# ZJU-FAST-Lab/uneven_planner

Measured on AMD Instinct MI355X. Metric: MINCO traj-opts/sec (batch), higher is better.
Workload: dtype f64

## Files before the change

### include/uneven_hip.h

```cpp
#ifndef UNEVEN_HIP_H
#define UNEVEN_HIP_H

#include <stdint.h>

#ifdef __cplusplus
extern "C" {
#endif

typedef struct uph_map uph_map;
typedef struct uph_ctx uph_ctx;
typedef struct uph_kino uph_kino;
typedef struct uph_body_layer uph_body_layer;

#define UPH_OK 0
#define UPH_ERR_INVALID (-1)
#define UPH_ERR_HIP (-2)
#define UPH_ERR_NO_DEVICE (-3)
#define UPH_ERR_LIMIT (-4)
#define UPH_ERR_NO_CACHE (-5)

#define UPH_RET_STOPPED 3
#define UPH_RET_UNSUPPORTED 4

#define UPH_RET_LEFT_TILE 5
// ... 115 lines not shown
int uph_map_create(const uph_map_params* mp, int device, uph_map** out);
int uph_map_create_f32(const uph_map_params* mp, int device, uph_map** out);
int uph_map_storage_bytes(const uph_map* m);
int uph_map_create_tile(const uph_map_params* mp, int device, int32_t x0, int32_t x1, int32_t f32, uph_map** out);
int uph_map_tile(const uph_map* m, int32_t* x0, int32_t* x1);
int uph_map_fill_fbm(uph_map* m, const uph_fbm_params* fp, int32_t x0, int32_t x1);
int uph_fbm_table(const uph_fbm_params* fp, double* table);
int uph_map_get_window(uph_map* m, int32_t x0, int32_t x1, int32_t y0, int32_t y1, double* rxs2);
void uph_map_destroy(uph_map* m);
int uph_map_dims(const uph_map* m, int32_t dims3[3]);
int uph_map_set_cells(uph_map* m, const double* rxs2);
int uph_map_get_cells(uph_map* m, double* rxs2, double* c, char* occ, char* occ_r2);
int uph_map_save_csv(const char* path, const double* rxs2, const int32_t dims3[3]);
int uph_map_load_csv(const char* path, const int32_t dims3[3], double* rxs2, double* c, int64_t* n_lines);
int uph_map_save_bin(const char* path, const double* rxs2, const int32_t dims3[3]);
int uph_map_load_bin(const char* path, const int32_t dims3[3], double* rxs2);
int uph_map_save_cache(uph_map* m, const char* csv_path, const char* bin_path);
int uph_map_load_cache(uph_map* m, const char* csv_path, const char* bin_path, int32_t* source);
int uph_map_build(uph_map* m, const float* xyz, int64_t n, int32_t x0, int32_t x1);
int uph_map_build_filtered(uph_map* m, const float* xyz, int64_t n, int32_t x0, int32_t x1);
typedef struct uph_map_update_info {
    int32_t dirty[4];
    int32_t changed[4];
    int32_t n_refit;
    int32_t n_far;
    int32_t n_changed;
    int32_t full_refit;
    int64_t n_removed, n_added, n_cloud;
} uph_map_update_info;
int uph_map_update(uph_map* m, const float box[4], const float* xyz, int64_t n, uph_map_update_info* info);
int uph_map_update_rect(const uph_map_params* mp, const float box[4], int32_t rect[4]);
int uph_map_update_stages(uph_map* m, double* out6);
int uph_map_build_multi(uph_map* const* maps, int32_t n_gpus, const float* xyz, int64_t n);
int uph_multi_slab_plan(int32_t nx, int32_t n_gpus, int32_t* x0, int32_t* x1, int32_t* per, int32_t* in_place);
int uph_map_fill_fbm_multi(uph_map* const* maps, int32_t n_gpus, const uph_fbm_params* fp);
int uph_map_multi_stats(uph_map* lead, double* fit_ms, double* exchange_ms, double* commit_ms, double* exchange_device_ms, int32_t* via_rccl);
int uph_rccl_selftest(int32_t n_devices, char* info, int32_t info_cap);
void uph_multi_shutdown(void);

int uph_map_cells_device(uph_map* m, void** dptr, int64_t* nbytes);
int uph_map_commit(uph_map* m);
int uph_map_export_slab_dev(uph_map* m, int32_t x0, int32_t x1, void* dst_dev);
int uph_map_import_cells_dev(uph_map* m, const void* src_dev);
int uph_terrain_query(uph_map* m, const double* pos, int32_t n, double* values7, double* grads21);
int uph_frontend_query(uph_map* m, const double* pos, int32_t n, double* sigma, int32_t* occ, int32_t* occ_xy);
int uph_terrain_pose_query(uph_map* m, const double* pos, int32_t n, double* pose12);
int uph_frontend_query_ms(uph_map* m, double* kernel_ms);
int64_t uph_map_filter_cloud(const float* xyz, int64_t n, float* out_xyz, int64_t cap);
int uph_map_build_stats(uph_map* m, double* kernel_ms, int64_t* cell_iters, int64_t* cloud_points);
int uph_map_build_stages(uph_map* m, double* out6);
int64_t uph_map_built_cloud(uph_map* m, float* out_xyz, int64_t cap);

int uph_kino_create(uph_map* m, const uph_kino_params* kp, int32_t slots, uph_kino** out);
void uph_kino_destroy(uph_kino* k);
int uph_kino_slots(const uph_kino* k);
int uph_kino_set_wps(uph_kino* k, int32_t wps);
int uph_kino_set_flags(uph_kino* k, int32_t flags);
int uph_kino_primitives(const uph_kino* k);
int uph_kino_plan_batch(uph_kino* k, int32_t B, const double* starts, const double* goals, int32_t path_cap, double* paths, int32_t* n_path, int32_t* status,
                        int32_t* iter_num, int32_t* use_node_num, int32_t max_expand, int32_t exp_cap, int32_t* expanded);
int uph_kino_stats(uph_kino* k, double* kernel_ms);

#define UPH_PLAN_PATH_CAP 1024
int uph_plan_upload(uph_kino* k, uph_ctx* c, const uph_manager_params* mp, int32_t B, const double* starts, const double* goals, int32_t path_cap,
                    int32_t* status, int32_t* traj_of, int32_t* n_inner_xy, int32_t* n_inner_yaw);
int uph_replan_upload(uph_kino* k, uph_ctx* src, uph_ctx* dst, const uph_manager_params* mp, int32_t B, const int32_t* src_traj, const double* t_switch,
                      const double* goals, int32_t path_cap, double* switch_states, int32_t* status, int32_t* traj_of, int32_t* n_inner_xy, int32_t* n_inner_yaw);
int uph_traj_states(uph_ctx* c, int32_t n, const int32_t* traj, const double* t, double* out10);
#define UPH_REFINE_AT_END 7
int uph_refine_upload(uph_ctx* src, uph_ctx* dst, int32_t B, const int32_t* src_traj, const double* t_switch, double* switch_states ,
                      int32_t* status, int32_t* traj_of, int32_t* n_inner_xy, int32_t* n_inner_yaw);
int uph_plan_staged(uph_ctx* c, int32_t cap_xy, int32_t cap_yaw, double* init_xy, double* end_xy, double* init_yaw, double* end_yaw, double* inner_xy,
                    double* inner_yaw, int32_t* n_inner_xy, int32_t* n_inner_yaw, double* total_time);

int uph_ctx_create(uph_map* m, const uph_opt_params* p, uph_ctx** out);
void uph_ctx_destroy(uph_ctx* c);
int uph_ctx_set_lanes(uph_ctx* c, int32_t lanes);
int uph_ctx_set_xcd_locality(uph_ctx* c, int32_t group);
int uph_ctx_set_wps(uph_ctx* c, int32_t wps);
int uph_ctx_set_sample_precision(uph_ctx* c, int32_t bits);
int uph_ctx_set_rho(uph_ctx* c, double rho);
int uph_ctx_get_rho(uph_ctx* c, double* rho);
int uph_ctx_set_trial_abandon(uph_ctx* c, int32_t on);

int uph_ctx_set_trace(uph_ctx* c, int32_t cap);
int uph_ctx_get_trace(uph_ctx* c, double* out);

int uph_optimize_batch(uph_ctx* c, int32_t B, const uph_problem* probs, uph_result* results);
int uph_optimize_batch_multi(uph_ctx* const* ctxs, int32_t n_gpus, int32_t B, const uph_problem* probs, uph_result* results);
int uph_multi_batch_plan(int32_t n_gpus, int32_t B, const uph_problem* probs, int32_t* share_of, double* predicted_cost);
int uph_batch_count(const uph_ctx* c);
int uph_batch_origin(const uph_ctx* c, int32_t* idx);
int uph_batch_upload(uph_ctx* c, int32_t B, const uph_problem* probs);
int uph_batch_solve(uph_ctx* c);
int uph_batch_solve_async(uph_ctx* c);
int uph_batch_wait(uph_ctx* c);
int uph_batch_download(uph_ctx* c, uph_result* results);
int uph_batch_stats(uph_ctx* c, double* kernel_ms, int64_t* evals, int64_t* sample_evals, int64_t* lbfgs_iters, int64_t* hist_bytes);
int uph_batch_abandon_stats(uph_ctx* c, int64_t* out5);

int uph_batch_prepare_ms(uph_ctx* c, double* ms);

int uph_batch_cycles(uph_ctx* c, long long* out);

int uph_eval_batch(uph_ctx* c, const double* x_packed, double* f, double* grad_packed, int32_t repeat);
int uph_penalty_batch(uph_ctx* c, int32_t repeat, int32_t store_residuals, double* cost, double* gdcxy_packed, double* gdcyaw_packed, double* gdT2);
int uph_init_scaling_batch(uph_ctx* c);
int uph_microbench_batch(uph_ctx* c, int32_t reps);
int uph_batch_set_state(uph_ctx* c, const double* lambda, const double* mu, const double* scale_cx, const double* scale_fx, const double* rho);
int uph_batch_set_x(uph_ctx* c, const double* x_packed);
int uph_batch_alm_passes(uph_ctx* c, int32_t max_passes);
int uph_batch_set_lbfgs_state(uph_ctx* c, const double* g, const double* d, const double* pf, const double* lm_s, const double* lm_y, const double* lm_ys, const double* scal5);
int uph_batch_lbfgs_resume(uph_ctx* c, int32_t budget, int32_t finish_pass);
int uph_batch_get_lbfgs_state(uph_ctx* c, double* g, double* d, double* pf, double* lm_s, double* lm_y, double* lm_ys, double* scal8);
int uph_report_batch(uph_ctx* c, double* out7);

#define UPH_ROLLOUT_STATE 1
#define UPH_ROLLOUT_TERRAIN 2
#define UPH_ROLLOUT_POSE 4
#define UPH_ROLLOUT_ALL 7
#define UPH_ROLLOUT_MAX_SAMPLES 262144
int uph_rollout_sizes(int32_t B, const int32_t* n_xy, const double* T_xy, const int32_t* n_yaw, const double* T_yaw, double dt, int32_t with_end,
                      int64_t* offsets);
int uph_rollout_plan(uph_ctx* c, double dt, int32_t with_end, int64_t* offsets);
int uph_rollout_batch(uph_ctx* c, double dt, int32_t with_end, int32_t channels, int32_t b0, int32_t b1, double* out);
int uph_rollout_batch_dev(uph_ctx* c, double dt, int32_t with_end, int32_t channels, int32_t b0, int32_t b1, void* out_dev);

#define UPH_CHECK_OCC_BIT 7
int uph_check_limits(const uph_ctx* c, double* lim7);
int uph_check_window(double dt, int32_t with_end, double total, double t_from, double t_to, int32_t* q_lo, int32_t* q_hi, int32_t* end_row);
int uph_check_batch(uph_ctx* c, int32_t n, const int32_t* traj, const double* t_from, const double* t_to , double dt, int32_t with_end,
                    const double* lim7 , double* first_t , int32_t* first_mask ,
                    int32_t* counts , double* worst , double* worst_t );
int uph_check_kernel_ms(const uph_ctx* c, double* kernel_ms);

int uph_locate_batch(uph_ctx* c, int32_t n, const int32_t* traj, const double* poses , const double* t_from, const double* t_to ,
                     double dt, int32_t with_end, double* near_t , double* near_d2 , int32_t* count , double* t ,
                     int32_t* refined , double* state , double* d2 , double* err );
int uph_within_batch(uph_ctx* c, int32_t n, const int32_t* traj, const double* rects , const double* t_from, const double* t_to ,
                     double dt, int32_t with_end, double* enter_t , double* leave_t , int32_t* counts );
int uph_locate_kernel_ms(const uph_ctx* c, double* kernel_ms);

int uph_separation_times(double t_from, double t_to, double dt, int64_t* K);
int uph_extent_batch(uph_ctx* c, int32_t n, const int32_t* traj, const double* t0, const double* t_from, const double* t_to, double dt,
                     double* box , int32_t* counts );
int uph_separation_batch(uph_ctx* ca, uph_ctx* cb , int32_t n, const int32_t* traj_a, const int32_t* traj_b, const double* t0_a, const double* t0_b,
                         const double* t_from, const double* t_to, double dt, const double* radius, double* min_d2 , double* min_t ,
                         double* first_t , double* last_t , int32_t* counts );
int uph_conflict_candidates(int32_t n, const double* box , const double* radius , int64_t cap, int32_t* pairs , int64_t* n_pairs);
int uph_conflicts_batch(uph_ctx* c, int32_t n, const int32_t* traj, const double* t0, const double* radius , double t_from, double t_to, double dt,
                        int64_t cap, int32_t* pairs , double* rows , int32_t* below ,
                        int64_t* n_conflicts, int64_t* n_candidates);
int uph_separation_kernel_ms(const uph_ctx* c, double* kernel_ms);

int uph_footprint_radii(int32_t n, const double* shape , const double* margin , double* r );
int uph_footprint_separation_batch(uph_ctx* ca, uph_ctx* cb , int32_t n, const int32_t* traj_a, const int32_t* traj_b, const double* t0_a,
                                   const double* t0_b, const double* t_from, const double* t_to, double dt, const double* shape_a ,
                                   const double* shape_b , const double* margin , double* min_c2 , double* min_t ,
                                   double* first_t , double* last_t , int32_t* counts );
int uph_footprint_conflicts_batch(uph_ctx* c, int32_t n, const int32_t* traj, const double* t0, const double* shape ,
                                  const double* margin , double t_from, double t_to, double dt, int64_t cap, int32_t* pairs ,
                                  double* rows , int32_t* below , int64_t* n_conflicts,
                                  int64_t* n_candidates);
int uph_footprint_kernel_ms(const uph_ctx* c, double* kernel_ms);

#define UPH_FOOT_OCC_XY 1
#define UPH_FOOT_OCC_YAW 2
#define UPH_FOOT_OUTSIDE 4
#define UPH_FOOT_ALL 7
int uph_footprint_check_columns(const uph_map_params* mp, int32_t n, const double* shape , const double* margin ,
                                int64_t* cols );
int uph_footprint_check_batch(uph_ctx* c, int32_t n, const int32_t* traj, const double* t_from, const double* t_to , double dt, int32_t with_end,
                              const double* shape , const double* margin , int32_t layers, double* first_t ,
                              double* last_t , int32_t* first_mask , int32_t* first_cell , int32_t* counts ,
                              int64_t* cells );
int uph_footprint_check_kernel_ms(const uph_ctx* c, double* kernel_ms);

#define UPH_BODY_MAX_R 64
int uph_body_stencil(const uph_map_params* mp, const double* shape , double margin, int32_t* R, int32_t* nyaw, double* cs, int32_t* lo,
                     int32_t* hi);
int uph_body_layer_margin(const uph_map_params* mp, const double* shape , double* margin);
int uph_body_layer_create(uph_map* m, const double* shape , double margin, int32_t layers, uph_body_layer** out);
// ... 67 lines not shown
```

### uneven_planner_amd/_lib.py

```python
import ctypes as C
import os

_HERE = os.path.dirname(os.path.abspath(__file__))
LIB_PATH = os.environ.get("UNEVENHIP_LIB") or os.path.join(_HERE, "libunevenhip.so")


class MapParams(C.Structure):
    _fields_ = [("iter_num", C.c_int32), ("map_size_x", C.c_double), ("map_size_y", C.c_double),
                ("ellipsoid_x", C.c_double), ("ellipsoid_y", C.c_double), ("ellipsoid_z", C.c_double),
                ("xy_resolution", C.c_double), ("yaw_resolution", C.c_double), ("min_cnormal", C.c_double),
                ("max_rho", C.c_double), ("gravity", C.c_double)]


class OptParams(C.Structure):
    _fields_ = [("rho_T", C.c_double), ("rho_ter", C.c_double), ("max_vel", C.c_double), ("max_acc_lon", C.c_double),
                ("max_acc_lat", C.c_double), ("max_kap", C.c_double), ("min_cxi", C.c_double), ("max_sig", C.c_double),
                ("use_scaling", C.c_int32), ("rho", C.c_double), ("beta", C.c_double), ("gamma", C.c_double),
                ("epsilon_con", C.c_double), ("max_iter", C.c_double), ("g_epsilon", C.c_double),
                ("min_step", C.c_double), ("inner_max_iter", C.c_double), ("delta", C.c_double),
                ("mem_size", C.c_int32), ("past", C.c_int32), ("int_K", C.c_int32)]


class ManagerParams(C.Structure):
    _fields_ = [("piece_len", C.c_double), ("mean_vel", C.c_double), ("init_time_times", C.c_double), ("yaw_piece_times", C.c_double),
# ... 18 lines not shown
                ("full_refit", C.c_int32), ("n_removed", C.c_int64), ("n_added", C.c_int64), ("n_cloud", C.c_int64)]


FBM_MAX_WAVES = 48
FBM_TABLE_DOUBLES = 4 * FBM_MAX_WAVES + 12 + 9
DP = C.POINTER(C.c_double)


class Problem(C.Structure):
    _fields_ = [("n_inner_xy", C.c_int32), ("n_inner_yaw", C.c_int32), ("init_xy", C.c_double * 6),
                ("end_xy", C.c_double * 6), ("init_yaw", C.c_double * 3), ("end_yaw", C.c_double * 3),
                ("inner_xy", DP), ("inner_yaw", DP), ("total_time", C.c_double)]


class Result(C.Structure):
    _fields_ = [("ret_code", C.c_int32), ("alm_iters", C.c_int32), ("lbfgs_iters", C.c_int32), ("evals", C.c_int32),
                ("last_lbfgs_ret", C.c_int32), ("cost", C.c_double), ("jerk_cost", C.c_double),
                ("piece_T_xy", C.c_double), ("piece_T_yaw", C.c_double), ("rho_final", C.c_double),
                ("scale_fx", C.c_double), ("x_final", DP), ("c_xy", DP), ("c_yaw", DP), ("hx", DP), ("gx", DP),
                ("lambda_", DP), ("mu", DP), ("scale_cx", DP)]


_VP = C.c_void_p
_I32, _I64 = C.c_int32, C.c_int64
SYMBOLS = {
    "uph_last_error": (C.c_char_p, []),
    "uph_device_count": (C.c_int, []),
    "uph_version": (C.c_char_p, []),
    "uph_resample_batch": (C.c_int, [C.POINTER(ManagerParams), _I32, DP, C.POINTER(_I64), _I32, _I32, DP, DP, DP, DP, DP, DP, C.POINTER(_I32), C.POINTER(_I32), DP, DP]),
    "uph_map_create": (C.c_int, [C.POINTER(MapParams), C.c_int, C.POINTER(_VP)]),
    "uph_map_create_f32": (C.c_int, [C.POINTER(MapParams), C.c_int, C.POINTER(_VP)]),
    "uph_map_storage_bytes": (C.c_int, [_VP]),
    "uph_map_create_tile": (C.c_int, [C.POINTER(MapParams), C.c_int, _I32, _I32, _I32, C.POINTER(_VP)]),
    "uph_map_tile": (C.c_int, [_VP, C.POINTER(_I32), C.POINTER(_I32)]),
    "uph_map_fill_fbm": (C.c_int, [_VP, C.POINTER(FbmParams), _I32, _I32]),
    "uph_fbm_table": (C.c_int, [C.POINTER(FbmParams), DP]),
    "uph_map_get_window": (C.c_int, [_VP, _I32, _I32, _I32, _I32, DP]),
    "uph_map_save_csv": (C.c_int, [C.c_char_p, DP, C.POINTER(_I32)]),
    "uph_map_load_csv": (C.c_int, [C.c_char_p, C.POINTER(_I32), DP, DP, C.POINTER(_I64)]),
    "uph_map_save_bin": (C.c_int, [C.c_char_p, DP, C.POINTER(_I32)]),
    "uph_map_load_bin": (C.c_int, [C.c_char_p, C.POINTER(_I32), DP]),
    "uph_map_save_cache": (C.c_int, [_VP, C.c_char_p, C.c_char_p]),
    "uph_map_load_cache": (C.c_int, [_VP, C.c_char_p, C.c_char_p, C.POINTER(_I32)]),
    "uph_map_destroy": (None, [_VP]),
    "uph_map_dims": (C.c_int, [_VP, C.POINTER(_I32)]),
    "uph_map_set_cells": (C.c_int, [_VP, DP]),
    "uph_map_get_cells": (C.c_int, [_VP, DP, DP, C.c_char_p, C.c_char_p]),
    "uph_map_build": (C.c_int, [_VP, C.POINTER(C.c_float), _I64, _I32, _I32]),
    "uph_map_build_filtered": (C.c_int, [_VP, C.POINTER(C.c_float), _I64, _I32, _I32]),
    "uph_map_update": (C.c_int, [_VP, C.POINTER(C.c_float), C.POINTER(C.c_float), _I64, C.POINTER(MapUpdateInfo)]),
    "uph_map_update_rect": (C.c_int, [C.POINTER(MapParams), C.POINTER(C.c_float), C.POINTER(_I32)]),
    "uph_map_update_stages": (C.c_int, [_VP, DP]),
    "uph_map_build_multi": (C.c_int, [C.POINTER(_VP), _I32, C.POINTER(C.c_float), _I64]),
    "uph_map_fill_fbm_multi": (C.c_int, [C.POINTER(_VP), _I32, C.POINTER(FbmParams)]),
    "uph_multi_slab_plan": (C.c_int, [_I32, _I32, C.POINTER(_I32), C.POINTER(_I32), C.POINTER(_I32), C.POINTER(_I32)]),
    "uph_multi_batch_plan": (C.c_int, [_I32, _I32, C.POINTER(Problem), C.POINTER(_I32), DP]),
    "uph_map_multi_stats": (C.c_int, [_VP, DP, DP, DP, DP, C.POINTER(_I32)]),
    "uph_multi_shutdown": (None, []),
    "uph_rccl_selftest": (C.c_int, [_I32, C.c_char_p, _I32]),
    "uph_optimize_batch_multi": (C.c_int, [C.POINTER(_VP), _I32, _I32, C.POINTER(Problem), C.POINTER(Result)]),
    "uph_batch_count": (C.c_int, [_VP]),
    "uph_batch_origin": (C.c_int, [_VP, C.POINTER(_I32)]),
    "uph_map_cells_device": (C.c_int, [_VP, C.POINTER(_VP), C.POINTER(_I64)]),
    "uph_map_commit": (C.c_int, [_VP]),
    "uph_map_export_slab_dev": (C.c_int, [_VP, _I32, _I32, _VP]),
    "uph_map_import_cells_dev": (C.c_int, [_VP, _VP]),
    "uph_terrain_query": (C.c_int, [_VP, DP, _I32, DP, DP]),
    "uph_frontend_query": (C.c_int, [_VP, DP, _I32, DP, C.POINTER(C.c_int32), C.POINTER(C.c_int32)]),
    "uph_terrain_pose_query": (C.c_int, [_VP, DP, _I32, DP]),
    "uph_frontend_query_ms": (C.c_int, [_VP, DP]),
    "uph_map_filter_cloud": (_I64, [C.POINTER(C.c_float), _I64, C.POINTER(C.c_float), _I64]),
    "uph_map_build_stats": (C.c_int, [_VP, DP, C.POINTER(_I64), C.POINTER(_I64)]),
    "uph_map_build_stages": (C.c_int, [_VP, DP]),
    "uph_map_built_cloud": (_I64, [_VP, C.POINTER(C.c_float), _I64]),
    "uph_ctx_create": (C.c_int, [_VP, C.POINTER(OptParams), C.POINTER(_VP)]),
    "uph_ctx_destroy": (None, [_VP]),
    "uph_ctx_set_lanes": (C.c_int, [_VP, _I32]),
    "uph_ctx_set_wps": (C.c_int, [_VP, _I32]),
    "uph_ctx_set_xcd_locality": (C.c_int, [_VP, _I32]),
    "uph_ctx_set_sample_precision": (C.c_int, [_VP, _I32]),
    "uph_ctx_set_rho": (C.c_int, [_VP, C.c_double]),
    "uph_ctx_get_rho": (C.c_int, [_VP, DP]),
    "uph_ctx_set_trial_abandon": (C.c_int, [_VP, _I32]),
    "uph_ctx_set_trace": (C.c_int, [_VP, _I32]),
    "uph_ctx_get_trace": (C.c_int, [_VP, DP]),
    "uph_optimize_batch": (C.c_int, [_VP, _I32, C.POINTER(Problem), C.POINTER(Result)]),
    "uph_batch_upload": (C.c_int, [_VP, _I32, C.POINTER(Problem)]),
    "uph_batch_solve": (C.c_int, [_VP]),
    "uph_batch_solve_async": (C.c_int, [_VP]),
    "uph_batch_wait": (C.c_int, [_VP]),
    "uph_batch_download": (C.c_int, [_VP, C.POINTER(Result)]),
    "uph_batch_stats": (C.c_int, [_VP, DP, C.POINTER(_I64), C.POINTER(_I64), C.POINTER(_I64), C.POINTER(_I64)]),
    "uph_batch_prepare_ms": (C.c_int, [_VP, DP]),
    "uph_batch_abandon_stats": (C.c_int, [_VP, C.POINTER(_I64)]),
    "uph_batch_cycles": (C.c_int, [_VP, C.POINTER(C.c_longlong)]),
    "uph_build_id": (C.c_char_p, []),
    "uph_eval_batch": (C.c_int, [_VP, DP, DP, DP, _I32]),
    "uph_penalty_batch": (C.c_int, [_VP, _I32, _I32, DP, DP, DP, DP]),
    "uph_init_scaling_batch": (C.c_int, [_VP]),
    "uph_microbench_batch": (C.c_int, [_VP, _I32]),
    "uph_batch_set_state": (C.c_int, [_VP, DP, DP, DP, DP, DP]),
    "uph_report_batch": (C.c_int, [_VP, DP]),
    "uph_rollout_sizes": (C.c_int, [_I32, C.POINTER(_I32), DP, C.POINTER(_I32), DP, C.c_double, _I32, C.POINTER(_I64)]),
    "uph_rollout_plan": (C.c_int, [_VP, C.c_double, _I32, C.POINTER(_I64)]),
    "uph_rollout_batch": (C.c_int, [_VP, C.c_double, _I32, _I32, _I32, _I32, DP]),
    "uph_rollout_batch_dev": (C.c_int, [_VP, C.c_double, _I32, _I32, _I32, _I32, _VP]),
    "uph_batch_set_x": (C.c_int, [_VP, DP]),
    "uph_batch_alm_passes": (C.c_int, [_VP, _I32]),
    "uph_batch_set_lbfgs_state": (C.c_int, [_VP, DP, DP, DP, DP, DP, DP, DP]),
    "uph_batch_lbfgs_resume": (C.c_int, [_VP, _I32, _I32]),
    "uph_batch_get_lbfgs_state": (C.c_int, [_VP, DP, DP, DP, DP, DP, DP, DP]),
    "uph_kino_create": (C.c_int, [_VP, C.POINTER(KinoParams), _I32, C.POINTER(_VP)]),
    "uph_kino_destroy": (None, [_VP]),
    "uph_kino_slots": (C.c_int, [_VP]),
    "uph_kino_set_wps": (C.c_int, [_VP, _I32]),
    "uph_kino_set_flags": (C.c_int, [_VP, _I32]),
    "uph_kino_primitives": (C.c_int, [_VP]),
    "uph_kino_plan_batch": (C.c_int, [_VP, _I32, DP, DP, _I32, DP, C.POINTER(_I32), C.POINTER(_I32), C.POINTER(_I32), C.POINTER(_I32), _I32, _I32, C.POINTER(_I32)]),
    "uph_kino_stats": (C.c_int, [_VP, DP]),
    "uph_plan_upload": (C.c_int, [_VP, _VP, C.POINTER(ManagerParams), _I32, DP, DP, _I32, C.POINTER(_I32), C.POINTER(_I32), C.POINTER(_I32), C.POINTER(_I32)]),
    "uph_plan_staged": (C.c_int, [_VP, _I32, _I32, DP, DP, DP, DP, DP, DP, C.POINTER(_I32), C.POINTER(_I32), DP]),
    "uph_replan_upload": (C.c_int, [_VP, _VP, _VP, C.POINTER(ManagerParams), _I32, C.POINTER(_I32), DP, DP, _I32, DP, C.POINTER(_I32), C.POINTER(_I32),
                                    C.POINTER(_I32), C.POINTER(_I32)]),
    "uph_traj_states": (C.c_int, [_VP, _I32, C.POINTER(_I32), DP, DP]),
    "uph_refine_upload": (C.c_int, [_VP, _VP, _I32, C.POINTER(_I32), DP, DP, C.POINTER(_I32), C.POINTER(_I32), C.POINTER(_I32), C.POINTER(_I32)]),
    "uph_check_limits": (C.c_int, [_VP, DP]),
    "uph_check_window": (C.c_int, [C.c_double, _I32, C.c_double, C.c_double, C.c_double, C.POINTER(_I32), C.POINTER(_I32), C.POINTER(_I32)]),
    "uph_check_batch": (C.c_int, [_VP, _I32, C.POINTER(_I32), DP, DP, C.c_double, _I32, DP, DP, C.POINTER(_I32), C.POINTER(_I32), DP, DP]),
    "uph_check_kernel_ms": (C.c_int, [_VP, DP]),
    "uph_locate_batch": (C.c_int, [_VP, _I32, C.POINTER(_I32), DP, DP, DP, C.c_double, _I32, DP, DP, C.POINTER(_I32), DP, C.POINTER(_I32), DP, DP, DP]),
    "uph_within_batch": (C.c_int, [_VP, _I32, C.POINTER(_I32), DP, DP, DP, C.c_double, _I32, DP, DP, C.POINTER(_I32)]),
    "uph_locate_kernel_ms": (C.c_int, [_VP, DP]),
    "uph_separation_times": (C.c_int, [C.c_double, C.c_double, C.c_double, C.POINTER(_I64)]),
    "uph_extent_batch": (C.c_int, [_VP, _I32, C.POINTER(_I32), DP, DP, DP, C.c_double, DP, C.POINTER(_I32)]),
    "uph_separation_batch": (C.c_int, [_VP, _VP, _I32, C.POINTER(_I32), C.POINTER(_I32), DP, DP, DP, DP, C.c_double, DP, DP, DP, DP, DP, C.POINTER(_I32)]),
    "uph_conflict_candidates": (C.c_int, [_I32, DP, DP, _I64, C.POINTER(_I32), C.POINTER(_I64)]),
    "uph_conflicts_batch": (C.c_int, [_VP, _I32, C.POINTER(_I32), DP, DP, C.c_double, C.c_double, C.c_double, _I64, C.POINTER(_I32), DP, C.POINTER(_I32),
                                      C.POINTER(_I64), C.POINTER(_I64)]),
    "uph_separation_kernel_ms": (C.c_int, [_VP, DP]),
    "uph_footprint_radii": (C.c_int, [_I32, DP, DP, DP]),
    "uph_footprint_separation_batch": (C.c_int, [_VP, _VP, _I32, C.POINTER(_I32), C.POINTER(_I32), DP, DP, DP, DP, C.c_double, DP, DP, DP, DP, DP, DP, DP,
                                                 C.POINTER(_I32)]),
    "uph_footprint_conflicts_batch": (C.c_int, [_VP, _I32, C.POINTER(_I32), DP, DP, DP, C.c_double, C.c_double, C.c_double, _I64, C.POINTER(_I32), DP,
                                                C.POINTER(_I32), C.POINTER(_I64), C.POINTER(_I64)]),
    "uph_footprint_kernel_ms": (C.c_int, [_VP, DP]),
    "uph_footprint_check_columns": (C.c_int, [C.POINTER(MapParams), _I32, DP, DP, C.POINTER(_I64)]),
    "uph_footprint_check_batch": (C.c_int, [_VP, _I32, C.POINTER(_I32), DP, DP, C.c_double, _I32, DP, DP, _I32, DP, DP, C.POINTER(_I32), C.POINTER(_I32),
                                            C.POINTER(_I32), C.POINTER(_I64)]),
    "uph_footprint_check_kernel_ms": (C.c_int, [_VP, DP]),
    "uph_delay_times": (C.c_int, [C.c_double, C.c_double, _I32, DP]),
    "uph_delay_levels": (C.c_int, [_I32, _I64, C.POINTER(_I32), C.POINTER(_I32)]),
    "uph_delay_sweep_batch": (C.c_int, [_VP, _VP, _I32, C.POINTER(_I32), C.POINTER(_I32), DP, DP, DP, DP, C.c_double, DP, C.c_double, C.c_double, _I32, DP, DP,
                                        C.POINTER(_I32), C.POINTER(_I32), C.POINTER(_I32)]),
    "uph_delay_extent_batch": (C.c_int, [_VP, _I32, C.POINTER(_I32), DP, DP, DP, C.c_double, C.c_double, C.c_double, _I32, DP, C.POINTER(_I32)]),
    "uph_delays_batch": (C.c_int, [_VP, _I32, C.POINTER(_I32), DP, DP, C.POINTER(_I32), C.c_double, C.c_double, C.c_double, C.c_double, C.c_double, _I32,
                                   C.POINTER(_I32), DP, C.POINTER(_I32), C.POINTER(_I64), C.POINTER(_I32), C.POINTER(_I32)]),
    "uph_footprint_delay_sweep_batch": (C.c_int, [_VP, _VP, _I32, C.POINTER(_I32), C.POINTER(_I32), DP, DP, DP, DP, C.c_double, DP, DP, DP, C.c_double, C.c_double,
                                                  _I32, DP, DP, C.POINTER(_I32), C.POINTER(_I32), C.POINTER(_I32), C.POINTER(_I32)]),
    "uph_footprint_delays_batch": (C.c_int, [_VP, _I32, C.POINTER(_I32), DP, DP, DP, C.POINTER(_I32), C.c_double, C.c_double, C.c_double, C.c_double, C.c_double,
                                             _I32, C.POINTER(_I32), DP, C.POINTER(_I32), C.POINTER(_I64), C.POINTER(_I32), C.POINTER(_I32)]),
    "uph_delay_kernel_ms": (C.c_int, [_VP, DP]),
    "uph_fleet_bytes": (C.c_int, [_I32, _I32, _I32, C.POINTER(_I64)]),
    "uph_fleet_create": (C.c_int, [_VP, C.POINTER(OptParams), _I32, _I32, _I32, C.POINTER(_VP)]),
    "uph_fleet_adopt": (C.c_int, [_VP, _VP, _I32, C.POINTER(_I32), C.POINTER(_I32), DP]),
    "uph_fleet_release": (C.c_int, [_VP, _I32, C.POINTER(_I32)]),
    "uph_fleet_info": (C.c_int, [_VP, C.POINTER(_I32), C.POINTER(_I32), C.POINTER(_I32), C.POINTER(_I32), DP]),
    "uph_fleet_get": (C.c_int, [_VP, _I32, C.POINTER(_I32), C.POINTER(_I32), C.POINTER(_I32), DP, DP, C.POINTER(_I32), DP, DP]),
    "uph_fleet_kernel_ms": (C.c_int, [_VP, DP]),
    "uph_body_stencil": (C.c_int, [C.POINTER(MapParams), DP, C.c_double, C.POINTER(_I32), C.POINTER(_I32), DP, C.POINTER(_I32), C.POINTER(_I32)]),
    "uph_body_layer_margin": (C.c_int, [C.POINTER(MapParams), DP, DP]),
    "uph_body_layer_create": (C.c_int, [_VP, DP, C.c_double, _I32, C.POINTER(_VP)]),
    "uph_body_layer_build": (C.c_int, [_VP]),
    "uph_body_layer_update": (C.c_int, [_VP, C.POINTER(_I32)]),
    "uph_body_layer_get": (C.c_int, [_VP, C.c_char_p]),
    "uph_body_layer_set": (C.c_int, [_VP, C.c_char_p]),
    "uph_body_layer_info": (C.c_int, [_VP, DP, DP, C.POINTER(_I32), C.POINTER(_I32), C.POINTER(_I32), C.POINTER(_I32)]),
    "uph_body_layer_kernel_ms": (C.c_int, [_VP, DP]),
# ... 100 lines not shown
```

### uneven_planner_amd/alm_traj_opt.py

```python
import ctypes as C

import numpy as np

from . import _lib

HILL_OPT_PARAMS = dict(rho_T=100000.0, rho_ter=10.0, max_vel=0.5, max_acc_lon=5.0, max_acc_lat=10.0, max_kap=2.1,
                       min_cxi=0.8, max_sig=0.05, use_scaling=True, rho=1.0, beta=1000.0, gamma=1.0,
                       epsilon_con=0.001, max_iter=10.0, g_epsilon=1.0e-3, min_step=1.0e-32, inner_max_iter=10000.0,
                       delta=1.0e-4, mem_size=256, past=3, int_K=16)
_INT_FIELDS = ("use_scaling", "mem_size", "past", "int_K")


def pack_problems(probs, int_K=16, with_sizes=False):
    arr = (_lib.Problem * len(probs))()
    keep, sizes = [], []
    for i, pr in enumerate(probs):
        ixy = np.ascontiguousarray(np.asarray(pr["inner_xy"], dtype=np.float64).T)
        iyw = np.ascontiguousarray(pr["inner_yaw"], dtype=np.float64)
        keep += [ixy, iyw]
        a = arr[i]
        a.n_inner_xy, a.n_inner_yaw = ixy.shape[0], iyw.shape[0]
        a.init_xy[:] = np.asarray(pr["init_xy"], dtype=np.float64).T.ravel().tolist()
        a.end_xy[:] = np.asarray(pr["end_xy"], dtype=np.float64).T.ravel().tolist()
        a.init_yaw[:] = np.asarray(pr["init_yaw"], dtype=np.float64).ravel().tolist()
# ... 515 lines not shown
    level = np.zeros(n, dtype=np.int32)
    for j, i in sorted(map(tuple, pairs[:, ::-1].tolist())):
        level[j] = max(level[j], level[i] + 1)
    return level


def delay_schedule(sweep, pairs, n, n_delays=None, order=None):
    pairs = np.asarray(pairs, dtype=np.int64).reshape(-1, 2)
    ahead = [[] for _ in range(n)]
    for h, i in sorted(map(tuple, pairs.tolist())):
        ahead[i].append(h)
    choice, blocker = np.zeros(n, dtype=np.int32), np.full(n, -1, dtype=np.int32)
    placed = np.zeros(n, dtype=bool)
    for i in (range(n) if order is None else order):
        assert all(placed[h] for h in ahead[i]), "delay_schedule: a vehicle ahead of %d is not placed yet" % i
        placed[i] = True
        if not ahead[i]:
            continue
        below = np.stack([np.asarray(sweep(h, max(int(choice[h]), 0), i)) for h in ahead[i]])
        nd = below.shape[1] if n_delays is None else int(n_delays[i])
        clear = np.nonzero((below[:, :nd] == 0).all(axis=0))[0]
        if clear.size:
            choice[i] = clear[0]
        else:
            choice[i] = -1
            blocker[i] = ahead[i][int(np.nonzero(below[:, 0] > 0)[0][0])]
    return dict(choice=choice, blocker=blocker)


class ALMTrajOpt:
    def __init__(self, uneven_map=None, params=None):
        self.L = _lib.load()
        q = dict(HILL_OPT_PARAMS)
        if params:
            q.update(params)
        for k, v in q.items():
            setattr(self, k, v)
        self._pnames = list(q.keys())
        self.h = None
        self.uneven_map = None
        self.in_opt = False
        self._B = 0
        self._sizes = []
        self._last = []
        if uneven_map is not None:
            self.setEnvironment(uneven_map)

    def __del__(self):
        try:
            if self.h:
                self.L.uph_ctx_destroy(self.h)
                self.h = None
        except Exception:
            pass

    def setEnvironment(self, env):
        self.uneven_map = env
        if self.h:
            self.L.uph_ctx_destroy(self.h)
            self.h = None
        p = _lib.OptParams(**{k: (int(getattr(self, k)) if k in _INT_FIELDS else float(getattr(self, k))) for k in self._pnames})
        h = C.c_void_p()
        _lib.check(self.L.uph_ctx_create(env.h, C.byref(p), C.byref(h)), "uph_ctx_create")
        self.h = h

    def set_lanes(self, lanes):
        _lib.check(self.L.uph_ctx_set_lanes(self.h, int(lanes)), "uph_ctx_set_lanes")

    def set_xcd_locality(self, group):
        _lib.check(self.L.uph_ctx_set_xcd_locality(self.h, int(group)), "uph_ctx_set_xcd_locality")

    def set_wps(self, wps):
        _lib.check(self.L.uph_ctx_set_wps(self.h, int(wps)), "uph_ctx_set_wps")

    def set_sample_precision(self, bits):
        _lib.check(self.L.uph_ctx_set_sample_precision(self.h, int(bits)), "uph_ctx_set_sample_precision")

    def set_rho(self, rho):
        _lib.check(self.L.uph_ctx_set_rho(self.h, float(rho)), "uph_ctx_set_rho")

    def set_trial_abandon(self, on):
        _lib.check(self.L.uph_ctx_set_trial_abandon(self.h, 1 if on else 0), "uph_ctx_set_trial_abandon")

    def get_rho(self):
        r = C.c_double(0)
        _lib.check(self.L.uph_ctx_get_rho(self.h, C.byref(r)), "uph_ctx_get_rho")
        return r.value

    def _make_problems(self, probs):
        arr, keep, self._sizes = pack_problems(probs, int(self.int_K), with_sizes=True)
        return arr, keep

    def upload(self, probs):
        arr, keep = self._make_problems(probs)
        self._B = 0
        _lib.check(self.L.uph_batch_upload(self.h, len(probs), arr), "uph_batch_upload")
        self._B = len(probs)
        self._trace_cap_up = getattr(self, "_trace_cap", 0)

    def solve(self):
        _lib.check(self.L.uph_batch_solve(self.h), "uph_batch_solve")

    def solve_async(self):
        _lib.check(self.L.uph_batch_solve_async(self.h), "uph_batch_solve_async")

    def wait(self):
        _lib.check(self.L.uph_batch_wait(self.h), "uph_batch_wait")

    def stats(self):
        ms = C.c_double(0)
        v = [C.c_int64(0) for _ in range(4)]
        _lib.check(self.L.uph_batch_stats(self.h, C.byref(ms), *[C.byref(x) for x in v]), "uph_batch_stats")
        pm = C.c_double(0)
        _lib.check(self.L.uph_batch_prepare_ms(self.h, C.byref(pm)), "uph_batch_prepare_ms")
        ab = (C.c_int64 * 5)()
        _lib.check(self.L.uph_batch_abandon_stats(self.h, ab), "uph_batch_abandon_stats")
        return dict(kernel_ms=ms.value, prepare_ms=pm.value, evals=v[0].value, sample_evals=v[1].value, lbfgs_iters=v[2].value, hist_bytes=v[3].value,
                    ls_rejected=ab[0], ls_guarded=ab[1], ls_abandoned=ab[2], chunks_skipped=ab[3], adjoints_skipped=ab[4])

    def cycles(self):
        out = np.zeros((max(0, self.L.uph_batch_count(self.h)), 16), dtype=np.int64)
        _lib.check(self.L.uph_batch_cycles(self.h, out.ctypes.data_as(C.POINTER(C.c_longlong))), "uph_batch_cycles")
        return out

    def origin(self):
        idx = np.zeros(max(0, self.L.uph_batch_count(self.h)), dtype=np.int32)
        _lib.check(self.L.uph_batch_origin(self.h, _ip(idx)), "uph_batch_origin")
        return idx

    def download(self, full=True):
        res, bufs = self._result_array(self._sizes, full)
        _lib.check(self.L.uph_batch_download(self.h, res), "uph_batch_download")
        self._last = self._collect(res, bufs)
        return self._last

    def optimize_batch(self, probs):
        self.upload(probs)
        self.solve()
        return self.download()

    def _result_array(self, sizes, full):
        res = (_lib.Result * len(sizes))()
        bufs = []
        for i, sz in enumerate(sizes):
            b = dict(x=np.zeros(sz["n"]), c_xy=np.zeros((6 * sz["Nxy"], 2)), c_yaw=np.zeros(6 * sz["Nyaw"]))
            r = res[i]
            r.x_final, r.c_xy, r.c_yaw = _dp(b["x"]), _dp(b["c_xy"]), _dp(b["c_yaw"])
            if full:
                b.update(hx=np.zeros(sz["S"]), gx=np.zeros(6 * sz["S"]), lam=np.zeros(sz["S"]), mu=np.zeros(6 * sz["S"]), scale_cx=np.zeros(7 * sz["S"]))
                r.hx, r.gx, r.lambda_, r.mu, r.scale_cx = _dp(b["hx"]), _dp(b["gx"]), _dp(b["lam"]), _dp(b["mu"]), _dp(b["scale_cx"])
            bufs.append(b)
        return res, bufs

    @staticmethod
    def _collect(res, bufs):
        out = []
        for i, b in enumerate(bufs):
            r = res[i]
            b.update(ret=r.ret_code, alm_iters=r.alm_iters, lbfgs_iters=r.lbfgs_iters, evals=r.evals, last_lbfgs_ret=r.last_lbfgs_ret,
                     cost=r.cost, jerk_cost=r.jerk_cost, T_xy=r.piece_T_xy, T_yaw=r.piece_T_yaw, rho_final=r.rho_final, scale_fx=r.scale_fx)
            out.append(b)
        return out

    def prepare_boundary(self, probs, full=False):
        arr, keep = self._make_problems(probs)
        res, bufs = self._result_array(self._sizes, full)
        return arr, keep, res, bufs

    def optimize_boundary(self, probs, full=False, prepared=None):
        arr, keep, res, bufs = prepared if prepared is not None else self.prepare_boundary(probs, full)
        self._B = 0
        import time
        t0 = time.perf_counter()
        rc = self.L.uph_optimize_batch(self.h, len(probs), arr, res)
        self.last_boundary_s = time.perf_counter() - t0
        _lib.check(rc, "uph_optimize_batch")
        self._B = len(probs)
        self._last = self._collect(res, bufs)
        return self._last

    @staticmethod
    def optimize_batch_multi(opts, probs, full=False):
        lead = opts[0]
        arr, keep = lead._make_problems(probs)
        sizes = list(lead._sizes)
        res, bufs = lead._result_array(sizes, full)
        hs = (C.c_void_p * len(opts))(*[o.h for o in opts])
        for o in opts:
            o._B, o._sizes, o._last = 0, [], None
        _lib.check(lead.L.uph_optimize_batch_multi(hs, len(opts), len(probs), arr, res), "uph_optimize_batch_multi")
        out = ALMTrajOpt._collect(res, bufs)
        for o in opts:
            n = o.L.uph_batch_count(o.h)
            if n <= 0:
                continue
            idx = o.origin()
            o._B, o._sizes, o._last = int(n), [sizes[i] for i in idx], [out[i] for i in idx]
        return out

    def plan_goals_upload(self, kino, starts, goals, path_cap=0, **manager_params):
        mp = self._manager_params("plan_goals", manager_params)
# ... 561 lines not shown
            self.L.uph_ctx_destroy(self.h)
            self.h = None
        p = _lib.OptParams(**{k: (int(getattr(self, k)) if k in _INT_FIELDS else float(getattr(self, k))) for k in self._pnames})
        h = C.c_void_p()
        _lib.check(self.L.uph_fleet_create(env.h, C.byref(p), self.slots, self.cap_xy, self.cap_yaw, C.byref(h)), "uph_fleet_create")
        self.h = h

    def adopt(self, src, src_traj, slot, t0=None):
        tr, sl, ts = _adopt_arrays(src_traj, slot, t0)
        if not isinstance(src, ALMTrajOpt) or src.h is None:
            raise _lib.UnevenHipError("adopt: src must be an ALMTrajOpt or a TrajFleet with a device context")
        _lib.check(self.L.uph_fleet_adopt(self.h, src.h, tr.shape[0], _ip(tr), _ip(sl), None if ts is None else _dp(ts)), "uph_fleet_adopt")

    def release(self, slot):
        sl = np.ascontiguousarray(slot, dtype=np.int32).reshape(-1)
        if sl.shape[0] == 0:
            raise _lib.UnevenHipError("release: no slot")
        _lib.check(self.L.uph_fleet_release(self.h, sl.shape[0], _ip(sl)), "uph_fleet_release")

    def _info(self):
        occ, t0 = np.zeros(self.slots, dtype=np.int32), np.zeros(self.slots)
        _lib.check(self.L.uph_fleet_info(self.h, None, None, None, _ip(occ), _dp(t0)), "uph_fleet_info")
        return occ.astype(bool), t0

    @property
    def occupied(self):
        return self._info()[0]

    @property
    def t0(self):
        return self._info()[1]

    def get(self, slot):
        sl = np.ascontiguousarray(slot, dtype=np.int32).reshape(-1)
        n = sl.shape[0]
        if n == 0:
            raise _lib.UnevenHipError("get: no slot")
        out = dict(n_xy=np.zeros(n, dtype=np.int32), n_yaw=np.zeros(n, dtype=np.int32), T_xy=np.zeros(n), T_yaw=np.zeros(n), ret=np.zeros(n, dtype=np.int32),
                   c_xy=np.zeros((n, 12 * self.cap_xy)), c_yaw=np.zeros((n, 6 * self.cap_yaw)))
        _lib.check(self.L.uph_fleet_get(self.h, n, _ip(sl), _ip(out["n_xy"]), _ip(out["n_yaw"]), _dp(out["T_xy"]), _dp(out["T_yaw"]), _ip(out["ret"]),
                                        _dp(out["c_xy"]), _dp(out["c_yaw"])), "uph_fleet_get")
        return out

    def getTraj(self, slot=0):
        g = self.get([int(slot)])
        if g["n_xy"][0] == 0:
            raise _lib.UnevenHipError("getTraj: slot %d of the fleet is empty" % int(slot))
        nx, ny = int(g["n_xy"][0]), int(g["n_yaw"][0])
        return SE2Traj(g["c_xy"][0, :12 * nx].reshape(-1, 2).copy(), g["c_yaw"][0, :6 * ny].copy(), float(g["T_xy"][0]), float(g["T_yaw"][0]))

    def adopt_kernel_ms(self):
        return self._kernel_ms("uph_fleet_kernel_ms")

    def _starts(self, traj, t0):
        return self.t0[np.ascontiguousarray(traj, dtype=np.int32).reshape(-1)] if t0 is None else t0

    def extent(self, traj, t_from, t_to, t0=None, dt=0.01):
        return super().extent(traj, t_from, t_to, t0=self._starts(traj, t0), dt=dt)

    def conflicts(self, traj, radius, t_from, t_to, t0=None, dt=0.05, cap=None):
        return super().conflicts(traj, radius, t_from, t_to, t0=self._starts(traj, t0), dt=dt, cap=cap)

    def footprint_conflicts(self, traj, shape, margin, t_from, t_to, t0=None, dt=0.05, cap=None):
        return super().footprint_conflicts(traj, shape, margin, t_from, t_to, t0=self._starts(traj, t0), dt=dt, cap=cap)

    def delay_extent(self, traj, t_from, t_to, delay0, delay_step, D, t0=None, dt=0.01):
        return super().delay_extent(traj, t_from, t_to, delay0, delay_step, D, t0=self._starts(traj, t0), dt=dt)

    def delays(self, traj, radius, t_from, t_to, delay0, delay_step, D, t0=None, n_delays=None, dt=0.05):
        return super().delays(traj, radius, t_from, t_to, delay0, delay_step, D, t0=self._starts(traj, t0), n_delays=n_delays, dt=dt)

    def footprint_delays(self, traj, shape, margin, t_from, t_to, delay0, delay_step, D, t0=None, n_delays=None, dt=0.05):
        return super().footprint_delays(traj, shape, margin, t_from, t_to, delay0, delay_step, D, t0=self._starts(traj, t0), n_delays=n_delays, dt=dt)


def _fleet_refuses(name):
    def method(self, *args, **kwargs):
        raise _lib.UnevenHipError("%s: a TrajFleet takes no upload, solve, evaluation, report, download or batch state (adopt() fills its slots)" % name)
    method.__name__ = name
    method.__doc__ = "refused on a TrajFleet"
    return method


FLEET_REFUSED = ("set_lanes", "set_xcd_locality", "set_wps", "set_sample_precision", "set_rho", "set_trial_abandon", "upload", "solve", "solve_async", "wait", "stats",
                 "cycles", "origin", "download", "optimize_batch", "prepare_boundary", "optimize_boundary", "plan_goals_upload", "plan_goals", "replan_goals_upload",
                 "replan_goals", "refine_upload", "refine", "plan_staged", "optimizeSE2Traj", "getTrajJerkCost", "getMaxVxAxAyCurAttSig", "x0_packed", "eval_batch",
                 "penalty_batch", "init_scaling_batch", "set_state", "set_x", "alm_passes", "set_lbfgs_state", "lbfgs_resume", "get_lbfgs_state", "set_trace", "get_trace")
for _name in FLEET_REFUSED:
    setattr(TrajFleet, _name, _fleet_refuses(_name))
del _name
```

### uneven_planner_amd/csrc/solver_program.hpp

```cpp
#pragma once
#include "terrain_dev.hpp"
#include "trajectory_dev.hpp"
#include "uph_common.hpp"

namespace uph {

#ifndef UPH_GRID_FROM_MEM
#define UPH_GRID_FROM_MEM 1
#endif
#ifndef UPH_PHASE_MASK
#define UPH_PHASE_MASK 15
#endif
#ifndef UPH_STATE_PROBE
#define UPH_STATE_PROBE(st) do { } while (0)
#endif
#ifndef UPH_SCALING_WB
#define UPH_SCALING_WB 8
#endif
#ifndef UPH_SC_XB
#define UPH_SC_XB 9
#endif
#ifndef UPH_SC_YB
#define UPH_SC_YB 14
#endif
#ifndef UPH_SC_WLO
#define UPH_SC_WLO 2
#endif
#ifndef UPH_SC_WHI
#define UPH_SC_WHI 3
#endif

#ifndef UPH_ASIDE_PREP
#define UPH_ASIDE_PREP 1
#endif
template <class WG, class F>
UPH_HD void asideKnotSolve(WG& wg, int lenW, int lenX, int n, F f) {
    (void)lenW; (void)lenX;
    wg.pfor(n, f);
}

#ifndef UPH_CHUNK_OVERLAP
#define UPH_CHUNK_OVERLAP 1
#endif
template <int M, class H, class WG, class C, class P>
UPH_HD void sampleChunk(WG& wg, int n, bool first, C compute, P commit) {
    (void)first;
    wg.template accChunk<M>(n, [&](int t, double* acc) { H h; compute(t, acc, h); commit(t, h); });
}
template <class WG, class F>
UPH_HD void pforOpen(WG& wg, int n, F f) { wg.pfor(n, f); }

template <class WG, class SR = double>
struct Solver {
    WG& wg;
    const GridDev& grid;
    const OptParams& P;
    const BatchDev& bd;
    const TrajDesc& td;
    int Nxy, Nyaw, n, S, K, mem, CH, CHP, recd;
    int CHS;
    int* rtag;
    double *x, *xp, *g, *gp, *d, *cxy, *cyaw, *Gxy, *Gyaw, *gamxy, *gamyaw, *bt, *rec, *wtab, *ttab, *pf, *hd;
    double* ab;
    int* abn;
    static constexpr int AB_DOUBLES = 4;
    double* up;
    static constexpr int UP_DOUBLES = 6;
    UPH_HD void tally(int k, bool yes) {
#if defined(__HIP_DEVICE_COMPILE__)
        if (yes && wg.wave == 0) abn[k] = abn[k] + 1;
#else
        if (yes) abn[k]++;
#endif
    }
    double *dual, *res, *scl, *hist;
    int hrow, hnp;
    const double *Wr_xy, *Wr_yaw;
    double rho, scale_fx, Txy, Tyaw, last_jerk, last_gd;
    long long hist_reads;
    long long cyc[16];
    long long t_last_eval_end;
    long long* sub_t = nullptr;
    int evals, bidx, trace_n;
    float inv_k1;
    double ec_irho, ec_step, ec_invK, ec_iTyaw, ec_omega, ec_omega_h;

    static constexpr int REC_FIELDS = 12;
    static UPH_HD size_t ldsDoubles(int Nxy, int Nyaw, int n, int CH, int mem, int K) {
        size_t recd = (size_t)REC_FIELDS * (CH + 1) + (CH + 1) / 2;
        const size_t nvec = 2 * (Nxy + 5) + (Nyaw + 5);
        const size_t knd = (size_t)knotBufDoubles(Nxy + 1, 4) + knotBufDoubles(Nyaw + 1, 2), adj = (size_t)knotBufDoubles(Nxy, 4) + knotBufDoubles(Nyaw, 2) + nvec;
        recd = recd < knd ? knd : recd;
        recd = recd < adj ? adj : recd;
        recd = recd < (size_t)mem ? (size_t)mem : recd;
        const size_t td_ = (size_t)Nxy + K + 2;
        return (size_t)5 * n + (nvec < td_ ? td_ : nvec) + 2 * (12 * Nxy + 6 * Nyaw) + recd + (size_t)6 * (K + 1) + THOMAS_DOUBLES + MAX_PAST + 8 + 18 + AB_DOUBLES + UP_DOUBLES;
    }

    UPH_HD Solver(WG& w, const GridDev& gr, const OptParams& p, const BatchDev& b, int bi, double* lds)
        : wg(w), grid(gr), P(p), bd(b), td(b.desc[bi]) {
        bidx = bi;
        Nxy = td.Nxy; Nyaw = td.Nyaw; n = td.n; S = td.S; K = P.int_K; mem = P.mem_size;
        inv_k1 = 1.0f / (float)(K + 1);
        CH = wg.size(); CHP = CH + 1; recd = REC_FIELDS * CHP + (CH + 1) / 2;
        CHS = CH;
#if !defined(UPH_ALIGNED_CHUNKS) || UPH_ALIGNED_CHUNKS
        {
            const int ppc = CH / (K + 1);
            if (ppc >= 1 && (Nxy + ppc - 1) / ppc == (S + CH - 1) / CH) CHS = ppc * (K + 1);
        }
#endif
        double* q = lds;
        x = q; q += n; g = q; q += n; d = q; q += n;
        xp = q; q += n; gp = q; q += n;
        const int nvec = 2 * (Nxy + 5) + (Nyaw + 5);
        bt = q;
        gamxy = q; gamyaw = q + 2 * (Nxy + 5);
        q += nvec < Nxy + K + 2 ? Nxy + K + 2 : nvec;
        cxy = q; q += 12 * Nxy; cyaw = q; q += 6 * Nyaw;
        Gxy = q; q += 12 * Nxy; Gyaw = q; q += 6 * Nyaw;
        wtab = q; q += 6 * (K + 1);
        rec = q;
        {
            size_t rd = (size_t)recd;
            const size_t knd = (size_t)knotBufDoubles(Nxy + 1, 4) + knotBufDoubles(Nyaw + 1, 2), adj = (size_t)knotBufDoubles(Nxy, 4) + knotBufDoubles(Nyaw, 2) + nvec;
            rd = rd < knd ? knd : rd; rd = rd < adj ? adj : rd; rd = rd < (size_t)mem ? (size_t)mem : rd;
            q += rd;
        }
        rtag = (int*)(rec + (size_t)REC_FIELDS * CHP);
        ttab = q; q += THOMAS_DOUBLES;
        pf = q; q += MAX_PAST + 8;
        hd = q; q += 18;
        ab = q; q += AB_DOUBLES;
        abn = (int*)(ab + 1);
        up = q; q += UP_DOUBLES;
        dual = bd.dual + 7 * td.off_s; res = bd.res + 7 * td.off_s; scl = bd.scl + 7 * td.off_s;
        hist = bd.hist + td.off_hist; hrow = histRowDoubles(n); hnp = 64 * histNQ(n);
        Wr_xy = bd.ops[td.op_xy].Wr; Wr_yaw = bd.ops[td.op_yaw].Wr;
        rho = 0; scale_fx = 1.0; Txy = Tyaw = 0; last_jerk = 0; hist_reads = 0; evals = 0; trace_n = 0;
        for (int q = 0; q < 16; q++) cyc[q] = 0;
        t_last_eval_end = 0;
        wg.pfor(18 + THOMAS_DOUBLES, [&](int t) {
            if (t == 0) { ab[0] = 0.0; abn[0] = abn[1] = abn[2] = abn[3] = 0; }
            if (t < 18) hd[t] = t < 6 ? td.init_xy[t] : (t < 12 ? td.end_xy[t - 6] : (t < 15 ? td.init_yaw[t - 12] : td.end_yaw[t - 15]));
            else ttab[t - 18] = bd.thomas[t - 18];
        });
    }

    UPH_HD void tracePush(double v) {
        if (bd.trace != nullptr && trace_n < bd.trace_cap) {
            const int at = trace_n;
            wg.one([&]() { bd.trace[(size_t)bidx * bd.trace_cap + at] = v; });
        }
        trace_n++;
    }

    static UPH_HD int divSmall(int a, int b, float inv) {
        int q = (int)((float)a * inv);
        const int r = a - q * b;
        if (r < 0) q--;
        else if (r >= b) q++;
        return q;
    }
    static UPH_HD int knotCol(int j, int N) { return j == 0 ? 0 : (j == N ? N + 2 : j + 2); }
    UPH_HD double knotPos(const double* xin, int j, int dd) const {
        if (dd < 2) return j == 0 ? hd[dd] : (j == Nxy ? hd[6 + dd] : xin[1 + 2 * (j - 1) + dd]);
        return j == 0 ? hd[12] : (j == Nyaw ? hd[15] : xin[1 + 2 * (Nxy - 1) + (j - 1)]);
    }

    UPH_HD double dot(const double* a, const double* b, int m) {
        double r[1];
        wg.template sum<1>(m, r, [&](int i, double* acc) { acc[0] += a[i] * b[i]; });
        return r[0];
    }
    UPH_HD double absmax(const double* a, int m) {
        return wg.maxv(m, [&](int i) { return fabs(a[i]); });
    }

    template <bool STEP>
    UPH_HD void generate(double* xin, double st) {
        UPH_MARK("generate");
        const long long tsub_start = wg.clock();
        const double tau_ = STEP ? fma(st, d[0], xp[0]) : xin[0];
        const double Ttot = expC2(tau_);
        Txy = wg.bcast(Ttot / (double)Nxy);
        Tyaw = wg.bcast(Ttot / (double)Nyaw);
#if !(UPH_ASIDE_PREP)
        ec_iTyaw = wg.bcast(1.0 / Tyaw);
#endif
        const double Tx = Txy, Ty = Tyaw;
        double* zxy = rec;
        double* zyaw = rec + knotBufDoubles(Nxy + 1, 4);
        wg.pfor(2 * (Nxy + 1) + (Nyaw + 1), [&](int t) {
            const bool isxy = t < 2 * (Nxy + 1);
            const int j = isxy ? (t >> 1) : t - 2 * (Nxy + 1), dd = isxy ? (t & 1) : 2, N = isxy ? Nxy : Nyaw, os = isxy ? 2 : 1;
            const double T1 = isxy ? Tx : Ty;
            const double* h0 = isxy ? hd + (dd & 1) : hd + 12;
            const double* h1 = isxy ? hd + 6 + (dd & 1) : hd + 15;
            double* z = isxy ? zxy + knotOffJ(j, 4) + (dd & 1) : zyaw + knotOffJ(j, 2);
            if (STEP && t == 0) xin[0] = tau_;
            if (j == 0) { z[0] = T1 * h0[os]; z[os] = T1 * T1 * h0[2 * os]; }
            else if (j == N) { z[0] = T1 * h1[os]; z[os] = T1 * T1 * h1[2 * os]; }
            else {
                double pm, p0, pp;
                if (STEP) {
                    const int ix = isxy ? 1 + 2 * (j - 1) + dd : 1 + 2 * (Nxy - 1) + (j - 1), ws = isxy ? 2 : 1;
                    p0 = fma(st, d[ix], xp[ix]);
                    pm = j == 1 ? h0[0] : fma(st, d[ix - ws], xp[ix - ws]);
                    pp = j == N - 1 ? h1[0] : fma(st, d[ix + ws], xp[ix + ws]);
                    xin[ix] = p0;
                } else { pm = knotPos(xin, j - 1, dd); p0 = knotPos(xin, j, dd); pp = knotPos(xin, j + 1, dd); }
                const double dp = pp - p0, dm = p0 - pm;
                double r0 = 20.0 * (dp - dm), r1 = -15.0 * (dp + dm);
                if (j == 1) { const double v0 = T1 * h0[os], a0 = T1 * T1 * h0[2 * os]; r0 += 8.0 * v0 + a0; r1 += 7.0 * v0 + a0; }
                if (j == N - 1) { const double vN = T1 * h1[os], aN = T1 * T1 * h1[2 * os]; r0 += -8.0 * vN + aN; r1 += 7.0 * vN - aN; }
                z[0] = r0; z[os] = r1;
            }
        });
        const long long tsub1 = wg.clock();
#if UPH_ASIDE_PREP
        asideKnotSolve(wg, Nyaw - 1, Nxy - 1, 2, [&](int t) {
            const double itx = 1.0 / Tx, ity = 1.0 / Ty, step = Tx / K, dtau = getTtoTauGrad(tau_);
            if (t == 0) { up[0] = itx; up[1] = ity; up[2] = step; up[3] = Ttot; up[4] = dtau; }
            const double add = t == 0 ? Tx : step;
            double* tab = t == 0 ? bt : bt + Nxy + 1;
            const int lim = t == 0 ? Nxy : K, top = Nxy > K ? Nxy : K;
// ... 549 lines not shown
            auto L1 = [&](int j) { return (j >= 1 && j <= N - 1) ? lam[knotOff(j - 1, ks) + cs] : 0.0; };
            double a = gdir[t], hT = 0.0;
            if (col == 1) { a += 8.0 * L0(1) + 7.0 * L1(1); hT = a * h0[cs]; }
            else if (col == 2) { a += L0(1) + L1(1); hT = a * (2.0 * T1 * h0[2 * cs]); }
            else if (col == N + 3) { a += -8.0 * L0(N - 1) + 7.0 * L1(N - 1); hT = a * h1[cs]; }
            else if (col == N + 4) { a += L0(N - 1) - L1(N - 1); hT = a * (2.0 * T1 * h1[2 * cs]); }
            else {
                const int k = col == 0 ? 0 : (col == N + 2 ? N : col - 2);
                a += 20.0 * ((L0(k - 1) - L0(k)) - (L0(k) - L0(k + 1))) - 15.0 * (L1(k - 1) - L1(k + 1));
            }
            if (isxy) gamxy[t] = a; else gamyaw[t - 2 * nbx] = a;
            acc[0] += isxy ? hT : 0.0;
            acc[1] += isxy ? 0.0 : hT;
            if (gout != nullptr && col >= 3 && col <= N + 1) {
                const int ix = isxy ? 1 + 2 * (col - 3) + dd : 1 + 2 * (Nxy - 1) + (col - 3);
                gout[ix] = a;
                acc[2] += a * d[ix];
            }
        });
        if (gd_out) *gd_out = hh[2];
        if (sub_t) { sub_t[4] += ta1 - ta0; sub_t[5] += ta2 - ta1; sub_t[6] += wg.clock() - ta2; }
        chain_xy = ch[0] + hh[0];
        chain_yaw = ch[1] + hh[1];
    }

    UPH_HD double evalStep() {
#if UPH_ASIDE_PREP
        return wg.bcast(up[2]);
#else
        return Txy / K;
#endif
    }
    UPH_HD void evalConsts(double step) {
        ec_irho = wg.bcast(1.0 / rho);
        ec_step = wg.bcast(step);
        ec_invK = wg.bcast(1.0 / K);
        ec_omega = wg.bcast(P.rho_ter * ec_step * scale_fx);
        ec_omega_h = wg.bcast(0.5 * P.rho_ter * ec_step * scale_fx);
    }

    UPH_HD void refreshResiduals() {
        UPH_MARK("refreshResiduals");
        wg.pfor(2, [&](int u) { fillTimes(u); });
        wg.pfor(S, [&](int s) { double dummy[3]; sampleEval<true>(s, 0, dummy); });
    }

    static constexpr double ABANDON_REL = 1e-9, ABANDON_REL_F = 1e-14;
    template <bool STEP>
    UPH_HD double eval(double* xin, double* gout, double st = 0.0, double thr = __builtin_huge_val()) {
        evals++;
        long long t0 = wg.clock();
        if (t_last_eval_end) cyc[5] += t0 - t_last_eval_end;
        if (UPH_PHASE_MASK & 1) generate<STEP>(xin, st);
        const double tau = wg.bcast(xin[0]);
        const double jw = wg.bcast(P.use_scaling ? scale_trick_jerk * scale_fx : scale_fx);
        double js[3] = {0.0, 0.0, 0.0};
        if (UPH_PHASE_MASK & 1) expand(xin, jw, js);
        long long t1 = wg.clock(); cyc[0] += t1 - t0;
        last_jerk = js[0];
        const double jerk_cost = wg.bcast(P.use_scaling ? js[0] * scale_fx * scale_trick_jerk : js[0] * scale_fx);
        evalConsts(evalStep());
        if (STEP && thr < __builtin_huge_val()) {
#if UPH_ASIDE_PREP
            double eq = wg.bcast(up[3]);
            pinv(eq);
            const double tau_lb = P.rho_T * eq * scale_fx;
#else
            double tq = tau;
            pinv(tq);
            const double tau_lb = P.rho_T * expC2(tq) * scale_fx;
#endif
            const double lbd = wg.bcast(ab[0]);
            const double L0 = wg.bcast(jerk_cost + tau_lb - lbd);
            const double mag = wg.bcast(fabs(jerk_cost) + fabs(tau_lb) + lbd);
            if (L0 > thr + ABANDON_REL * mag && L0 < __builtin_huge_val() && ec_omega >= 0.0) {
                tally(2, true);
                t_last_eval_end = wg.clock();
                return L0;
            }
        }
        double sm[3] = {0.0, 0.0, 0.0};
        wg.template accBegin<3>();
#if UPH_CHUNK_OVERLAP
        for (int s0 = 0; s0 < S; s0 += CHS) {
            const int cnt = S - s0 < CHS ? S - s0 : CHS;
            t0 = wg.clock();
            if (UPH_PHASE_MASK & 2)
                sampleChunk<3, SampleRec<SR>>(wg, cnt, s0 == 0, [&](int t, double* acc, SampleRec<SR>& h) { sampleCompute<0, SR>(s0 + t, acc, h); },
                                              [&](int t, const SampleRec<SR>& h) { sampleCommit<SR>(t, h); });
            t1 = wg.clock(); cyc[1] += t1 - t0;
            if (UPH_PHASE_MASK & 4) scatterChunk<false>(s0, cnt);
            cyc[2] += wg.clock() - t1;
        }
#else
        for (int s0 = 0; s0 < S; s0 += CHS) {
            const int cnt = S - s0 < CHS ? S - s0 : CHS;
            t0 = wg.clock();
            if (UPH_PHASE_MASK & 2) wg.template accChunk<3>(cnt, [&](int t, double* acc) { sampleEval<false, SR>(s0 + t, t, acc); });
            t1 = wg.clock(); cyc[1] += t1 - t0;
            if (UPH_PHASE_MASK & 4) scatterChunk(s0, cnt);
            cyc[2] += wg.clock() - t1;
        }
#endif
        wg.template accEnd<3>(sm);
        t1 = wg.clock();
        if (STEP && thr < __builtin_huge_val()) {
#if UPH_ASIDE_PREP
            double eq = wg.bcast(up[3]);
            pinv(eq);
            const double tau_q = P.rho_T * eq * scale_fx;
#else
            double tq = tau;
            pinv(tq);
            const double tau_q = P.rho_T * expC2(tq) * scale_fx;
#endif
            const double fq = wg.bcast(jerk_cost + sm[0] + tau_q);
            const double mag = wg.bcast(fabs(jerk_cost) + fabs(sm[0]) + fabs(tau_q));
            if (fq > thr + ABANDON_REL_F * mag && fq < __builtin_huge_val()) {
                tally(3, true);
                t_last_eval_end = wg.clock();
                return fq;
            }
        }
        double chx = 0.0, chy = 0.0, gdw = 0.0;
        if (UPH_PHASE_MASK & 8) adjoint(chx, chy, gout, &gdw);
        t0 = wg.clock(); cyc[3] += t0 - t1;
        const double gTx = js[1] * jw + sm[1] + chx;
        const double gTy = js[2] * jw + sm[2] + chy;
        const double grad_Tsum = P.rho_T * scale_fx + gTx / Nxy + gTy / Nyaw;
#if UPH_ASIDE_PREP
        const double g0 = wg.bcast(grad_Tsum * wg.bcast(up[4]));
        const double etau = wg.bcast(up[3]);
#else
        const double g0 = wg.bcast(grad_Tsum * getTtoTauGrad(tau));
        const double etau = expC2(tau);
#endif
        wg.pfor(1, [&](int) { gout[0] = g0; });
        last_gd = wg.bcast(gdw + g0 * d[0]);
        const double tau_cost = P.rho_T * etau * scale_fx;
        t_last_eval_end = wg.clock();
        return wg.bcast(jerk_cost + sm[0] + tau_cost);
    }

    UPH_HD void initScaling(double* x0) {
        generate<false>(x0, 0.0);
        const double tau = x0[0];
        const double dTau = getTtoTauGrad(tau);
        double js[3];
        expand(x0, 1.0, js);
        double sm[3] = {0.0, 0.0, 0.0};
        for (int s0 = 0; s0 < S; s0 += CHS) {
            const int cnt = S - s0 < CHS ? S - s0 : CHS;
            double part[3];
            wg.template sum<3>(cnt, part, [&](int t, double* acc) { sampleObjective(s0 + t, t, acc); });
            sm[0] += part[0]; sm[1] += part[1]; sm[2] += part[2];
            scatterChunk(s0, cnt);
        }
        double chx, chy;
        adjoint(chx, chy);
        const double gTau_fx = (P.rho_T + (js[1] + sm[1] + chx) / Nxy + (js[2] + sm[2] + chy) / Nyaw) * dTau;
        const double mq = wg.maxv((Nxy - 1) * 2 + (Nyaw - 1), [&](int t) {
            return t < (Nxy - 1) * 2 ? fabs(gamxy[3 * 2 + t]) : fabs(gamyaw[3 + (t - (Nxy - 1) * 2)]);
        });
        scale_fx = wg.bcast(1.0 / dmax(1.0, dmax(mq, fabs(gTau_fx))));
        wg.pfor(2, [&](int u) { fillTimes(u); });
        wg.pfor(S, [&](int s) { scalingSample(s, dTau); });
    }

    UPH_HD void scalingSample(int s, double dTau) {
        const int i = divSmall(s, K + 1, inv_k1), j = s - i * (K + 1);
        Kin k;
        kin(i, j, k);
// ... 115 lines not shown
                mx[q] = mq;
            }
        }
        double htx[NQS], hty[NQS];
        {
            const int sc[4] = {1, 2, Nxy + 3, Nxy + 4};
            double w[4][4];
#pragma unroll
            for (int u = 0; u < 4; u++) { w[0][u] = WL[sc[u]]; w[1][u] = WL[nbx + sc[u]]; w[2][u] = WR[sc[u]]; w[3][u] = WR[nbx + sc[u]]; }
#pragma unroll
            for (int q = 0; q < NQS; q++) {
                const double c00 = inL ? dvL[q][0] : 0.0, c01 = inL ? dvL[q][1] : 0.0, c10 = inL ? daL[q][0] : 0.0, c11 = inL ? daL[q][1] : 0.0;
                const double c20 = inR ? dvR[q][0] : 0.0, c21 = inR ? dvR[q][1] : 0.0, c30 = inR ? daR[q][0] : 0.0, c31 = inR ? daR[q][1] : 0.0;
                double a0[4], a1[4];
#pragma unroll
                for (int u = 0; u < 4; u++) {
                    a0[u] = (w[0][u] * c00 + w[1][u] * c10) + (w[2][u] * c20 + w[3][u] * c30);
                    a1[u] = (w[0][u] * c01 + w[1][u] * c11) + (w[2][u] * c21 + w[3][u] * c31);
                }
                if (!inL) { a0[0] += dvL[q][0]; a1[0] += dvL[q][1]; a0[1] += daL[q][0]; a1[1] += daL[q][1]; }
                if (!inR) { a0[2] += dvR[q][0]; a1[2] += dvR[q][1]; a0[3] += daR[q][0]; a1[3] += daR[q][1]; }
                double headtail_x = 0.0;
                headtail_x += a0[0] * hd[2] + a1[0] * hd[3];
                headtail_x += 2.0 * Tx * (a0[1] * hd[4] + a1[1] * hd[5]);
                headtail_x += a0[2] * hd[8] + a1[2] * hd[9];
                headtail_x += 2.0 * Tx * (a0[3] * hd[10] + a1[3] * hd[11]);
                htx[q] = headtail_x;
            }
        }
        const bool yL = m >= 1, yR = m + 1 <= Nyaw - 1;
        const auto VL = UPH_AS_GLOBAL(Wr_yaw + (size_t)(yL ? 2 * (m - 1) : 0) * nby);
        const auto VR = UPH_AS_GLOBAL(Wr_yaw + (size_t)(yR ? 2 * m : 0) * nby);
        const int qL = knotCol(m, Nyaw), qR = knotCol(m + 1, Nyaw);
        for (int c0 = 3; c0 < Nyaw + 2; c0 += UPH_SCALING_WB) {
            double w[4][UPH_SCALING_WB];
#pragma unroll
            for (int u = 0; u < UPH_SCALING_WB; u++) {
                const int cc = c0 + u < Nyaw + 2 ? c0 + u : Nyaw + 1;
                w[0][u] = VL[cc]; w[1][u] = VL[nby + cc]; w[2][u] = VR[cc]; w[3][u] = VR[nby + cc];
            }
#pragma unroll
            for (int q = 0; q < NQS; q++) {
                const double y0_ = yL ? yvL[q] : 0.0, y1_ = yL ? yaL[q] : 0.0, y2_ = yR ? yvR[q] : 0.0, y3_ = yR ? yaR[q] : 0.0;
                double mq = mx[q];
#pragma unroll
                for (int u = 0; u < UPH_SCALING_WB; u++) {
                    const int col = c0 + u;
                    double a0 = (w[0][u] * y0_ + w[1][u] * y1_) + (w[2][u] * y2_ + w[3][u] * y3_);
                    if (col == qL) a0 += ypL[q];
                    if (col == qR) a0 += ypR[q];
                    if (col < Nyaw + 2) mq = dmax(mq, fabs(a0));
                }
                mx[q] = mq;
            }
        }
        {
            const int sc[4] = {1, 2, Nyaw + 3, Nyaw + 4};
            double w[4][4];
#pragma unroll
            for (int u = 0; u < 4; u++) { w[0][u] = VL[sc[u]]; w[1][u] = VL[nby + sc[u]]; w[2][u] = VR[sc[u]]; w[3][u] = VR[nby + sc[u]]; }
#pragma unroll
            for (int q = 0; q < NQS; q++) {
                const double y0_ = yL ? yvL[q] : 0.0, y1_ = yL ? yaL[q] : 0.0, y2_ = yR ? yvR[q] : 0.0, y3_ = yR ? yaR[q] : 0.0;
                double a0[4];
#pragma unroll
                for (int u = 0; u < 4; u++) a0[u] = (w[0][u] * y0_ + w[1][u] * y1_) + (w[2][u] * y2_ + w[3][u] * y3_);
                if (!yL) { a0[0] += yvL[q]; a0[1] += yaL[q]; }
                if (!yR) { a0[2] += yvR[q]; a0[3] += yaR[q]; }
                double headtail_y = 0.0;
                headtail_y += a0[0] * hd[13];
                headtail_y += 2.0 * Ty * a0[1] * hd[14];
                headtail_y += a0[2] * hd[16];
                headtail_y += 2.0 * Ty * a0[3] * hd[17];
                hty[q] = headtail_y;
            }
        }
#pragma unroll
        for (int q = 0; q < NQS; q++) {
            const double gTau = ((sumx[q] + htx[q]) / Nxy + (sumy[q] + hty[q]) / Nyaw) * dTau;
            scl[(Q0 + q) * S + s] = 1.0 / dmax(1.0, dmax(mx[q], fabs(gTau)));
        }
    }

    UPH_HD bool abandonAllowed() const {
        if (sizeof(SR) != sizeof(double)) return false;
#if defined(__HIP_DEVICE_COMPILE__) && UPH_GRID_FROM_MEM
        typedef const __attribute__((address_space(4))) int* pi_t;
        pi_t pt = (pi_t)(const void*)&bd.params_mem->no_trial_abandon;
        asm volatile("" : "+s"(pt));
        return *pt == 0;
#else
        return P.no_trial_abandon == 0;
#endif
    }
    static UPH_HD bool noExitAfterRejection(int count, double stp, double mu, double stpmin, double stpmax, int max_linesearch, double machine_prec) {
        return count + 1 < max_linesearch && (stp - mu) >= machine_prec * stp && 0.5 * (mu + stp) >= stpmin && stp <= stpmax;
    }
    UPH_HD int lineSearch(double& f, double& stp, double stpmin, double stpmax, double dginit) {
        int count = 0;
        bool brackt = false, touched = false;
        double mu = 0.0, nu = stpmax;
        if (!(stp > 0.0)) return LBFGSERR_INVALIDPARAMETERS;
        if (0.0 < dginit) return LBFGSERR_INCREASEGRADIENT;
        const double finit = wg.bcast(f);
        const double dgtest = wg.bcast(P.f_dec_coeff * dginit);
        const double dstest = wg.bcast(P.s_curv_coeff * dginit);
        const bool on = abandonAllowed();
        const double pst = wg.bcast(P.past > 0 ? P.delta / P.past * (fabs(finit) + 1.0) : 0.0);
        while (true) {
            const double arm = stp * dgtest;
            const bool may = on && noExitAfterRejection(count, stp, mu, stpmin, stpmax, P.max_linesearch, P.machine_prec);
            const double thr = wg.bcast(may ? dmax(finit + arm, finit + pst) + ABANDON_REL * (fabs(finit) + fabs(arm) + pst) : __builtin_huge_val());
            f = eval<true>(x, g, stp, thr);
            ++count;
            if (isinf(f) || isnan(f)) return LBFGSERR_INVALID_FUNCVAL;
            if (P.past > 0 && fabs(finit - f) / (fabs(finit) + 1.0) < P.delta / P.past) return count;
            if (f > finit + stp * dgtest) {
                tally(0, on); tally(1, on && !may);
                nu = stp;
                brackt = true;
            } else {
                if (last_gd < dstest) mu = stp;
                else return count;
            }
            if (P.max_linesearch <= count) return LBFGSERR_MAXIMUMLINESEARCH;
            if (brackt && (nu - mu) < P.machine_prec * nu) return LBFGSERR_WIDTHTOOSMALL;
            if (brackt) stp = wg.bcast(0.5 * (mu + nu));
            else stp = wg.bcast(stp * 2.0);
            if (stp < stpmin) return LBFGSERR_MINIMUMSTEP;
            if (stp > stpmax) {
                if (touched) return LBFGSERR_MAXIMUMSTEP;
                touched = true;
                stp = stpmax;
            }
        }
    }

    struct ResumeIO { double step, fx; int k, end, bound, budget; };
    static constexpr int LBFGS_RUNNING_HOOK = 999;
    template <bool RESUME>
    UPH_HD int lbfgs(double& f_out, int& k_out, ResumeIO* io = nullptr) {
        int ret = 0, k = 0, ls, end = 0, bound = 0, budget = 0;
        double step = 0.0, fx = 0.0, ys, yy, dginit = 0.0;
        const int m = mem;
        bool run = true;
        if constexpr (RESUME) {
            step = io->step; fx = io->fx; k = io->k; end = io->end; bound = io->bound; budget = io->budget;
            wg.pfor(n, [&](int i) { xp[i] = x[i]; gp[i] = g[i]; });
            dginit = dot(g, d, n);
        } else {
            fx = eval<false>(x, g);
            wg.pfor(n + 1, [&](int i) { if (i < n) { d[i] = -g[i]; xp[i] = x[i]; gp[i] = g[i]; } else pf[0] = fx; });
            const double gnorm0 = absmax(g, n), xnorm0 = absmax(x, n);
            if (gnorm0 / dmax(1.0, xnorm0) < P.g_epsilon) {
                ret = LBFGS_CONVERGENCE;
                run = false;
            } else {
                const double dd0 = dot(d, d, n);
                step = 1.0 / sqrt(dd0);
                dginit = -dd0;
                k = 1; end = 0; bound = 0;
            }
        }
        double gnorm_inf, xnorm_inf;
        if (run) {
            while (true) {
                if constexpr (RESUME) {
                    if (budget == 0) { ret = LBFGS_RUNNING_HOOK; break; }
                    budget--;
                }
                ls = lineSearch(fx, step, P.min_step, P.max_step, dginit);
                if (ls < 0) {
                    wg.pfor(n, [&](int i) { x[i] = xp[i]; g[i] = gp[i]; });
                    ret = ls;
                    break;
                }
                tracePush(fx);
                if (k > 1000) { ret = LBFGS_CANCELED; break; }
                double* hr = hist + (size_t)end * hrow;
                double* sc = hr + 2;
                double* yc = hr + 2 + hnp;
                const double pf_old = (0 < P.past && P.past <= k) ? wg.bcast(pf[k % P.past]) : 0.0;
                UPH_MARK("lbfgs.bookkeeping");
                double r5[5], mx2[2];
                wg.template sumMax<5, 2>(n, r5, mx2, [&](int i, double* acc, double* mx) {
                    const double xv = x[i], gv = g[i], xo = xp[i], go = gp[i];
                    const double sv = xv - xo, yv = gv - go;
                    mx[0] = dmax(mx[0], fabs(gv)); mx[1] = dmax(mx[1], fabs(xv));
                    sc[i] = sv; yc[i] = yv;
                    acc[0] += yv * sv; acc[1] += yv * yv; acc[2] += sv * sv; acc[3] += go * go; acc[4] += gv * gv;
                    xp[i] = xv; gp[i] = gv;
                    d[i] = -gv;
                });
                gnorm_inf = mx2[0];
                xnorm_inf = mx2[1];
                if (gnorm_inf / dmax(1.0, xnorm_inf) < P.g_epsilon) { ret = LBFGS_CONVERGENCE; break; }
                if (0 < P.past) {
                    if (P.past <= k) {
                        const double rate = fabs(pf_old - fx) / dmax(1.0, fabs(fx));
                        if (rate < P.delta) { ret = LBFGS_STOP; break; }
                    }
                }
                if (P.inner_max_iter != 0 && P.inner_max_iter <= k) { ret = LBFGSERR_MAXIMUMITERATION; break; }
                ys = r5[0]; yy = r5[1];
                const double cau = r5[2] * sqrt(r5[3]) * P.cautious_factor;
                {
                    const int kk = k, e0 = end;
                    const double fv = fx, ysv = ys;
                    wg.pfor(1, [&](int) {
                        if (0 < P.past) pf[kk % P.past] = fv;
                        double* h0 = hist + (size_t)e0 * hrow;
                        h0[0] = ysv; h0[1] = 1.0 / ysv;
                    });
                }
                ++k;
                dginit = -r5[4];
                if (ys > cau) {
                    ++bound;
                    bound = m < bound ? m : bound;
                    end = (end + 1) % m;
                    const long long tq = wg.clock();
                    cyc[7] += tq - t_last_eval_end;
                    UPH_MARK("twoLoop");
                    wg.twoLoop(d, g, n, hist, pf + MAX_PAST, rec, m, end, bound, ys / yy);
                    dginit = wg.bcast(pf[MAX_PAST]);
                    t_last_eval_end = wg.clock();
                    cyc[4] += t_last_eval_end - tq;
                    hist_reads += (long long)4 * bound * n;
                }
                step = 1.0;
            }
        }
        if constexpr (RESUME) { io->step = step; io->fx = fx; io->k = k; io->end = end; io->bound = bound; }
        f_out = fx;
        k_out = k;
        return ret;
    }

    UPH_HD void setDualBound(double sq) {
        const double v = rho > 0.0 ? sq * (0.5 / rho) : __builtin_huge_val();
        wg.one([&]() { ab[0] = v; });
    }
    UPH_HD void formDualBound() {
        double sq[1];
        wg.template sum<1>(S, sq, [&](int s, double* acc) {
            double a = 0.0;
            for (int q = 0; q < 7; q++) { const double v = dual[q * S + s]; a += v * v; }
            acc[0] += a;
        });
        setDualBound(sq[0]);
    }
    UPH_HD void updateDualVars() {
        UPH_MARK("updateDualVars");
        const double r = rho;
        double sq[1];
        wg.template sum<1>(S, sq, [&](int s, double* acc) {
            dual[s] += r * res[s];
            for (int q = 1; q < 7; q++) dual[q * S + s] = dmax(dual[q * S + s] + r * res[q * S + s], 0.0);
            double a = 0.0;
            for (int q = 0; q < 7; q++) { const double v = dual[q * S + s]; a += v * v; }
            acc[0] += a;
        });
        rho = wg.bcast(dmin((1 + P.gamma) * rho, P.beta));
        setDualBound(sq[0]);
    }
    UPH_HD bool judgeConvergence() {
        const double r = rho;
        const double rh = wg.maxv(S, [&](int s) { return fabs(res[s]); });
        const double rg = wg.maxv(6 * S, [&](int t) { return fabs(dmax(res[S + t], -dual[S + t] / r)); });
        return dmax(rh, rg) < P.epsilon_con;
    }

    UPH_HD void storeTrajectory(TrajState& st) {
        double* oc = bd.cxy + td.off_cxy;
        double* oy = bd.cyaw + td.off_cyaw;
        wg.pfor(12 * Nxy + 6 * Nyaw, [&](int t) { if (t < 12 * Nxy) oc[t] = cxy[t]; else oy[t - 12 * Nxy] = cyaw[t - 12 * Nxy]; });
        wg.pfor(1, [&](int) {
            st.T_xy = Txy; st.T_yaw = Tyaw; st.jerk_cost = last_jerk; st.scale_fx = scale_fx; st.rho = rho;
            st.evals = evals; st.hist_reads = hist_reads;
            st.ls_rejected = abn[0]; st.ls_guarded = abn[1]; st.ls_abandoned = abn[2]; st.adjoints_skipped = abn[3] + abn[2];
            st.chunks_skipped = abn[2] * ((S + CHS - 1) / CHS);
#ifdef UPH_TL_PROF
            for (int q = 0; q < 6; q++) cyc[8 + q] = wg.tl[q];
#endif
            for (int q = 0; q < 16; q++) st.cyc[q] = cyc[q];
        });
        UPH_STATE_PROBE(st);
#ifdef UPH_BAR_PROF
        wg.sync();
        wg.dumpBar(&st.cyc[8]);
#endif
    }

    UPH_HD void prepare(TrajState& st) {
        const double* gx0 = bd.x0 + td.off_x;
        double* gx = bd.x + td.off_x;
        rho = wg.bcast(st.rho);
        scale_fx = 1.0;
        wg.pfor(S > n ? S : n, [&](int t) {
            if (t < n) { x[t] = gx0[t]; gx[t] = gx0[t]; }
            if (t < S) for (int q = 0; q < 7; q++) { dual[q * S + t] = 0.0; res[q * S + t] = 0.0; scl[q * S + t] = 1.0; }
        });
        const long long tstart = wg.clock();
        if (P.use_scaling) initScaling(x);
        cyc[5] += wg.clock() - tstart;
        wg.pfor(1, [&](int) { st.scale_fx = scale_fx; st.cyc[5] = cyc[5]; });
    }

    UPH_HD void optimize(TrajState& st, int cap = 0) {
        double* gx0 = bd.x + td.off_x;
        rho = wg.bcast(st.rho);
        scale_fx = wg.bcast(st.scale_fx);
        wg.pfor(n, [&](int t) { x[t] = gx0[t]; });
        formDualBound();
        const long long tstart = wg.clock();
        cyc[14] = wg.realtime();
        int ret_code = 0, iter = 0, total_k = 0, last_ret = 0;
        double inner_cost = 0.0;
        while (true) {
            int kk = 0;
            tracePush(-1.0);
            const int result = lbfgs<false>(inner_cost, kk);
            refreshResiduals();
            total_k += kk;
            last_ret = result;
            if (result == LBFGS_CONVERGENCE || result == LBFGS_CANCELED || result == LBFGS_STOP || result == LBFGSERR_MAXIMUMITERATION) {
            } else if (result == LBFGSERR_MAXIMUMLINESEARCH) {
            } else { ret_code = 1; break; }
            updateDualVars();
            if (judgeConvergence()) break;
            if (++iter > P.max_iter) { ret_code = 2; break; }
            if (cap > 0 && iter >= cap) { ret_code = 3; break; }
        }
        wg.pfor(n, [&](int t) { gx0[t] = x[t]; bd.gout[td.off_x + t] = g[t]; });
        cyc[6] = wg.clock() - tstart;
        cyc[15] = wg.realtime();
        storeTrajectory(st);
        wg.pfor(1, [&](int) {
            st.ret_code = ret_code; st.alm_iters = iter; st.lbfgs_iters = total_k; st.last_lbfgs_ret = last_ret; st.f = inner_cost;
        });
    }

    UPH_HD void resumeHook(TrajState& st, int budget, int finish) {
        double* gx = bd.x + td.off_x;
        double* gg = bd.gout + td.off_x;
        double* gd = bd.rs_d + td.off_x;
        double* rs = bd.rs + (size_t)bidx * 24;
        rho = wg.bcast(st.rho); scale_fx = wg.bcast(st.scale_fx);
        formDualBound();
        wg.pfor(n + MAX_PAST, [&](int t) { if (t < n) { x[t] = gx[t]; g[t] = gg[t]; d[t] = gd[t]; } else pf[t - n] = rs[8 + t - n]; });
        ResumeIO io;
        io.step = wg.bcast(rs[0]); io.fx = wg.bcast(rs[1]);
        io.k = (int)wg.bcast(rs[2]); io.end = (int)wg.bcast(rs[3]); io.bound = (int)wg.bcast(rs[4]); io.budget = budget;
        double f = 0.0;
        int kk = 0;
        const int ret = lbfgs<true>(f, kk, &io);
        int accepted = 0, conv = 0;
        if (evals > 0) refreshResiduals();
        if (finish && ret != LBFGS_RUNNING_HOOK) {
            accepted = (ret == LBFGS_CONVERGENCE || ret == LBFGS_CANCELED || ret == LBFGS_STOP || ret == LBFGSERR_MAXIMUMITERATION || ret == LBFGSERR_MAXIMUMLINESEARCH) ? 1 : 0;
            if (accepted) { updateDualVars(); conv = judgeConvergence() ? 1 : 0; }
        }
        wg.pfor(n + MAX_PAST, [&](int t) { if (t < n) { gx[t] = x[t]; gg[t] = g[t]; gd[t] = d[t]; } else rs[8 + t - n] = pf[t - n]; });
        wg.pfor(1, [&](int) {
// ... 158 lines not shown
```

### uneven_planner_amd/csrc/unevenhip.hip

```cpp
#include <hip/hip_runtime.h>

#include <type_traits>

#include <algorithm>
#include <cmath>
#include <cstdio>
#include <cstdlib>
#include <cstring>
#include <map>
#include <numeric>
#include <string>
#include <thread>
#include <vector>

#include "../../include/uneven_hip.h"
#include "minco_op_host.hpp"
#include "resample_walk.hpp"
#include "solver_program.hpp"
#include "uph_ctx.hpp"
#include "wave_dev.hpp"

using namespace uph;

#ifndef UPH_THOMAS_KPL
// ... 70 lines not shown
            const int jlo = pbase < 0 ? -pbase : 0;
            int jhi = cnt - pbase < K1 ? cnt - pbase : K1;
            if (pi >= P) jhi = 0;
            const double* rb = rec + dd * CHP + pbase;
            d4_t acc0 = {0.0, 0.0, 0.0, 0.0}, acc1 = {0.0, 0.0, 0.0, 0.0};
#pragma unroll
            for (int st = 0; st < (NQ + 3) / 4; st++) {
                const int q = 4 * st + kk;
                const int f = (q >= K1 ? 1 : 0) + (q >= 2 * K1 ? 1 : 0) + (q >= 3 * K1 ? 1 : 0);
                const int j = q - K1 * f;
                const double wv = wtab[6 * j + c - f];
                const double rv = rb[2 * f * CHP + j];
                const double cf = f == 0 ? 1.0 : (f == 1 ? c1 : c2);
                const double a = (c < 6 && c >= f && q < NQ) ? cf * wv : 0.0;
                const double b = (j >= jlo && j < jhi && q < NQ) ? rv : 0.0;
                if (st & 1) acc1 = __builtin_amdgcn_mfma_f64_16x16x4f64(a, b, acc1, 0, 0, 0);
                else acc0 = __builtin_amdgcn_mfma_f64_16x16x4f64(a, b, acc0, 0, 0, 0);
            }
            if (pi < P) {
                double* gp = Gxy + 12 * (i0 + pi) + dd;
                gp[2 * kk] += acc0[0] + acc1[0];
                if (kk < 2) gp[2 * (4 + kk)] += acc0[1] + acc1[1];
            }
        }
    }
    __device__ __forceinline__ void sync() { bar(0); }
    __device__ __forceinline__ int size() const { return NT; }
#ifndef UPH_CYC
#define UPH_CYC 0
#endif
#if UPH_CYC
    __device__ __forceinline__ long long clock() { return (long long)__builtin_readcyclecounter(); }
    __device__ __forceinline__ long long realtime() { return (long long)__builtin_amdgcn_s_memrealtime(); }
#else
    __device__ __forceinline__ long long clock() { return 0; }
    __device__ __forceinline__ long long realtime() { return 0; }
#endif
    template <class F>
    __device__ __forceinline__ void one(F f) { if (tid == 0) f(); }

    template <int M, class F>
    __device__ __forceinline__ void sum(int n, double* out, F f) {
        double acc[M];
#pragma unroll
        for (int m = 0; m < M; m++) acc[m] = 0.0;
        for (int i = ftid(); i < n; i += NT) f(i, acc);
#pragma unroll
        for (int m = 0; m < M; m++) acc[m] = waveSum(acc[m]);
        double* r = red + par * (NW * MAXM);
        par ^= 1;
        if (lane == 0) {
#pragma unroll
            for (int m = 0; m < M; m++) r[wave * MAXM + m] = acc[m];
        }
        bar(0);
#pragma unroll
        for (int m = 0; m < M; m++) {
            double t = r[m];
#pragma unroll
            for (int w = 1; w < NW; w++) t += r[w * MAXM + m];
            out[m] = uni(t);
        }
    }
    double pacc[MAXM];
    template <int M>
    __device__ __forceinline__ void accBegin() {
#pragma unroll
        for (int m = 0; m < M; m++) pacc[m] = 0.0;
    }
    template <int M, class F>
    __device__ __forceinline__ void accChunk(int n, F f) {
        for (int i = ftid(); i < n; i += NT) f(i, pacc);
        bar(0);
    }
    template <int M, class H, class C, class P>
    __device__ __forceinline__ void accChunkSplit(int n, bool first, C compute, P commit) {
        const int i = ftid();
        H h;
        if (i < n) compute(i, pacc, h);
        if (!first) bar(3);
        if (i < n) commit(i, h);
        bar(0);
    }
    template <int M>
    __device__ __forceinline__ void accEnd(double* out) {
        double acc[M];
#pragma unroll
        for (int m = 0; m < M; m++) acc[m] = waveSum(pacc[m]);
        double* r = red + par * (NW * MAXM);
        par ^= 1;
        if (lane == 0) {
#pragma unroll
            for (int m = 0; m < M; m++) r[wave * MAXM + m] = acc[m];
        }
        bar(0);
#pragma unroll
        for (int m = 0; m < M; m++) {
            double t = r[m];
#pragma unroll
            for (int w = 1; w < NW; w++) t += r[w * MAXM + m];
            out[m] = uni(t);
        }
    }
    template <int MS, int MM, class F>
    __device__ __forceinline__ void sumMax(int n, double* outS, double* outM, F f) {
        static_assert(MS + MM <= MAXM, "reduction scratch too small");
        double acc[MS], mx[MM];
#pragma unroll
        for (int m = 0; m < MS; m++) acc[m] = 0.0;
#pragma unroll
        for (int m = 0; m < MM; m++) mx[m] = 0.0;
        for (int i = ftid(); i < n; i += NT) f(i, acc, mx);
#pragma unroll
        for (int m = 0; m < MS; m++) acc[m] = waveSum(acc[m]);
#pragma unroll
        for (int m = 0; m < MM; m++) mx[m] = waveMax(mx[m]);
        double* r = red + par * (NW * MAXM);
        par ^= 1;
        if (lane == 0) {
#pragma unroll
            for (int m = 0; m < MS; m++) r[wave * MAXM + m] = acc[m];
#pragma unroll
            for (int m = 0; m < MM; m++) r[wave * MAXM + MS + m] = mx[m];
        }
        bar(0);
#pragma unroll
        for (int m = 0; m < MS; m++) {
            double t = r[m];
#pragma unroll
            for (int w = 1; w < NW; w++) t += r[w * MAXM + m];
            outS[m] = uni(t);
        }
#pragma unroll
        for (int m = 0; m < MM; m++) {
            double t = r[MS + m];
#pragma unroll
            for (int w = 1; w < NW; w++) t = r[w * MAXM + MS + m] > t ? r[w * MAXM + MS + m] : t;
            outM[m] = uni(t);
        }
    }
    __device__ __forceinline__ double bcast(double v) const { return uni(v); }
    static __device__ __forceinline__ double divByStored(double x, double ys, double r) {
        const double q0 = x * r;
        return fma(fma(-q0, ys, x), r, q0);
    }
    template <int NQ, int PF>
    __device__ __forceinline__ void twoLoopT(double* d, const double* g, double* dg_out, double* al_lds, int n_, const double* hist_, int m_, int end_, int bound_, double scale_) {
        typedef double dbl2_t __attribute__((ext_vector_type(2)));
        typedef const __attribute__((address_space(1))) char* gbytes;
        constexpr int NP2 = NQ / 2;
        constexpr bool ODD = (NQ & 1) != 0;
        constexpr int NPAD = 64 * NQ, ROWB = (2 + 2 * NPAD) * 8;
        const gbytes hist = (gbytes)uniG(hist_);
        const int lane = flane();
        const int n = uni(n_), m = uni(m_), end = uni(end_), bound = uni(bound_);
        const double scale = uni(scale_);
        const unsigned l16 = 16u * (unsigned)lane, l8 = 8u * (unsigned)lane;
        auto eidx = [&](int q) { return q < 2 * NP2 ? 128 * (q >> 1) + 2 * lane + (q & 1) : 64 * (NQ - 1) + lane; };
        double dr[NQ], sr[PF][NQ], yr[PF][NQ], ysr[PF], rysr[PF];
#pragma unroll
        for (int q = 0; q < NQ; q++) { const int e = eidx(q); dr[q] = e < n ? d[e] : 0.0; }
        auto fetch = [&](int slot, int j) {
            const gbytes row = hist + (size_t)((unsigned)j * (unsigned)ROWB);
            const dbl2_t yr2 = *(const __attribute__((address_space(1))) dbl2_t*)row;
            ysr[slot] = yr2.x; rysr[slot] = yr2.y;
#pragma unroll
// ... 177 lines not shown
            const double p0 = shl1(z0), p1 = shl1(z1);
            z0 = fma(F[0][1], p1, fma(F[0][0], p0, c[0][0]));
            z1 = fma(F[0][3], p1, fma(F[0][2], p0, c[0][1]));
        }
        {
            const double p0 = shl1(z0), p1 = shl1(z1);
#pragma unroll
            for (int k = 0; k < KPL; k++) {
                if (j0 + k <= len) {
                    pk[k * ks] = fma(F[k][1], p1, fma(F[k][0], p0, c[k][0]));
                    pk[k * ks + cs] = fma(F[k][3], p1, fma(F[k][2], p0, c[k][1]));
                }
            }
        }
    }
    template <bool ADJ>
    __device__ __forceinline__ void thomasT(const double* tab, double* bw, int lenW, double* bx, int lenX) {
        UPH_MARK("thomas");
        __builtin_amdgcn_s_setprio(3);
        const bool packed = uni(lenW) <= 32 * UPH_THOMAS_KPL - 1 && uni(lenX) <= 16 * UPH_THOMAS_KPL - 1;
        if (packed) {
            if (wave == 0) thomasWave<2, ADJ, UPH_THOMAS_KPL>(tab, bw, lenW, bx, lenX);
        } else if (NW >= 2) {
            if (wave == 0) thomasWave<0, ADJ, UPH_THOMAS_KPL>(tab, bw, lenW, bx, lenX);
            else if (wave == 1) thomasWave<1, ADJ, UPH_THOMAS_KPL>(tab, bw, lenW, bx, lenX);
        } else {
            thomasWave<0, ADJ, UPH_THOMAS_KPL>(tab, bw, lenW, bx, lenX);
            thomasWave<1, ADJ, UPH_THOMAS_KPL>(tab, bw, lenW, bx, lenX);
        }
        __builtin_amdgcn_s_setprio(0);
        bar(2);
    }
    template <class F>
    __device__ __forceinline__ void aside(int lenW, int lenX, int n, F f) {
        const bool packed = uni(lenW) <= 32 * UPH_THOMAS_KPL - 1 && uni(lenX) <= 16 * UPH_THOMAS_KPL - 1;
        const int aw = NW >= 2 && packed ? 1 : (NW >= 3 ? 2 : 0);
        if (wave == aw) {
            const int l = flane();
            if (l < n) f(l);
        }
    }
    __device__ __forceinline__ void thomas(const double* tab, bool adj, double* bw, int lenW, double* bx, int lenX) {
        if (adj) thomasT<true>(tab, bw, lenW, bx, lenX);
        else thomasT<false>(tab, bw, lenW, bx, lenX);
    }
    __device__ __forceinline__ void twoLoop(double* d, const double* g, int n, const double* __restrict__ hist, double* dg_out, double* al_lds, int m, int end, int bound, double scale) {
        if (wave == 0) {
            __builtin_amdgcn_s_setprio(3);
            constexpr int PF = UPH_TWOLOOP_PF;
            const int nq = uni((n + 63) >> 6);
            if (nq == 1) twoLoopT<1, PF>(d, g, dg_out, al_lds, n, hist, m, end, bound, scale);
            else if (nq == 2) twoLoopT<2, PF>(d, g, dg_out, al_lds, n, hist, m, end, bound, scale);
            else if (nq == 3) twoLoopT<3, PF>(d, g, dg_out, al_lds, n, hist, m, end, bound, scale);
            else if (nq == 4) twoLoopT<4, PF>(d, g, dg_out, al_lds, n, hist, m, end, bound, scale);
            else if (nq == 5) twoLoopT<5, 2>(d, g, dg_out, al_lds, n, hist, m, end, bound, scale);
            else if (nq == 6) twoLoopT<6, 2>(d, g, dg_out, al_lds, n, hist, m, end, bound, scale);
            else if (nq == 7) twoLoopT<7, 2>(d, g, dg_out, al_lds, n, hist, m, end, bound, scale);
            else twoLoopT<8, 2>(d, g, dg_out, al_lds, n, hist, m, end, bound, scale);
            __builtin_amdgcn_s_setprio(0);
        }
        bar(1);
    }
    template <class F>
    __device__ __forceinline__ double maxv(int n, F f) {
        double a = 0.0;
        for (int i = ftid(); i < n; i += NT) { const double v = f(i); a = v > a ? v : a; }
        a = waveMax(a);
        double* r = red + par * (NW * MAXM);
        par ^= 1;
        if (lane == 0) r[wave * MAXM] = a;
        bar(0);
        double t = r[0];
#pragma unroll
        for (int w = 1; w < NW; w++) t = r[w * MAXM] > t ? r[w * MAXM] : t;
        return uni(t);
    }
};

template <int NT, class F>
__device__ __forceinline__ void asideKnotSolve(DevWG<NT>& wg, int lenW, int lenX, int n, F f) { wg.aside(lenW, lenX, n, f); }

template <int M, class H, int NT, class C, class P>
__device__ __forceinline__ void sampleChunk(DevWG<NT>& wg, int n, bool first, C compute, P commit) { wg.template accChunkSplit<M, H>(n, first, compute, commit); }
template <int NT, class F>
__device__ __forceinline__ void pforOpen(DevWG<NT>& wg, int n, F f) { wg.pforOpen(n, f); }

template <int NT, int WPS, int MODE, bool F32S = false>
__global__ __launch_bounds__(NT, WPS) void uph_solver_kernel(GridDev grid, OptParams P, BatchDev bd, int repeat) {
    extern __shared__ double lds[];
    const int w = blockIdx.x;
    if (w >= bd.B) return;
    const int b = bd.order ? bd.order[w] : w;
    DevWG<NT> wg(lds);
    typedef typename std::conditional<F32S, f32r, double>::type SR;
    Solver<DevWG<NT>, SR> sol(wg, grid, P, bd, b, lds + DevWG<NT>::SCRATCH);
    TrajState& st = bd.state[b];
    if (MODE == 0) sol.evalOnly(st, repeat);
    else if (MODE == 1) sol.prepare(st);
    else if (MODE == 2) sol.optimize(st, repeat);
    else if (MODE == 7) sol.resumeHook(st, repeat >> 1, repeat & 1);
    else if (MODE == 8) { if (repeat & 1) sol.template penaltyOnly<true>(st, repeat >> 1); else sol.template penaltyOnly<false>(st, repeat >> 1); }
    else if (MODE == 3) sol.report(st);
    else if (MODE == 5) sol.microbench(st, repeat);
    else sol.scalingOnly(st);
}

__global__ void uph_fill_kernel(double* __restrict__ p, size_t n, double v) {
    for (size_t i = (size_t)blockIdx.x * blockDim.x + threadIdx.x; i < n; i += (size_t)gridDim.x * blockDim.x) p[i] = v;
}

__global__ void uph_terrain_kernel(GridDev grid, const double* __restrict__ pos, int n, double* __restrict__ values, double* __restrict__ grads) {
    const int i = blockIdx.x * blockDim.x + threadIdx.x;
    if (i >= n) return;
    const double yaw = pos[3 * i + 2];
    double v[7], g[7][3];
    terrainAllWithGrad(grid, pos[3 * i], pos[3 * i + 1], yaw, cos(yaw), sin(yaw), v, g);
    for (int k = 0; k < 7; k++) {
        values[7 * i + k] = v[k];
        for (int q = 0; q < 3; q++) grads[21 * i + 3 * k + q] = g[k][q];
    }
}

constexpr int PLAN_SX = UPH_MAX_PIECE_XY - 1, PLAN_SY = UPH_MAX_PIECE_YAW - 1;
struct PlanHead {
    int32_t n_inner_xy, n_inner_yaw;
    int32_t short_path, pad;
    double p_init[2], p_end[2];
    double yaw_init, yaw_end;
    double total_time;
    double lo[2], hi[2];
    double turn, kink;
};
struct PlanPath {
    const double* p;
    __host__ __device__ double operator()(int64_t k, int j) const { return p[3 * k + j]; }
};
struct PlanSink {
    double *oxy, *oyw;
    int nxy, nyw;
    double nlo[2], nhi[2], prev, turn, kink;
    __device__ void xy(double x, double y) {
        if (nxy < PLAN_SX) { oxy[2 * nxy] = x; oxy[2 * nxy + 1] = y; }
        nxy++;
        nlo[0] = x < nlo[0] ? x : nlo[0]; nlo[1] = y < nlo[1] ? y : nlo[1];
        nhi[0] = nhi[0] < x ? x : nhi[0]; nhi[1] = nhi[1] < y ? y : nhi[1];
    }
    __device__ void yaw(double v) {
        if (nyw < PLAN_SY) oyw[nyw] = v;
        nyw++;
        const double d = fabs(v - prev);
        turn += d; kink = kink < d ? d : kink; prev = v;
    }
    __device__ void unwrapped(int64_t, double) {}
};
__global__ __launch_bounds__(64) void uph_plan_resample_kernel(uph_manager_params mp, const double* __restrict__ paths, int path_cap, const int* __restrict__ n_path,
                                                               const int* __restrict__ status, int nq, const int* __restrict__ goal_of, double* __restrict__ st_xy,
                                                               double* __restrict__ st_yaw, PlanHead* __restrict__ heads) {
#pragma clang fp contract(off)
    const int q = blockIdx.x * blockDim.x + threadIdx.x;
    if (q >= nq) return;
    const int m = n_path[q];
    if (status[q] != UPH_KINO_OK || m > path_cap) return;
    const int g = goal_of ? goal_of[q] : q;
    PlanHead h = PlanHead{};
    if (m < 2) { h.short_path = 1; heads[g] = h; return; }
    const double* p = paths + (size_t)q * path_cap * 3;
// ... 283 lines not shown
int uph_device_count(void) {
    int n = 0;
    if (hipGetDeviceCount(&n) != hipSuccess) return 0;
    return n;
}

int uph_ctx_create(uph_map* m, const uph_opt_params* p, uph_ctx** out) {
    if (!m || !p || !out) { setError("uph_ctx_create: null argument"); return UPH_ERR_INVALID; }
    if (p->mem_size < 1 || p->mem_size > UPH_MAX_MEM || p->past < 0 || p->past > UPH_MAX_PAST || p->int_K < 1 || p->int_K > 64) {
        setError("uph_ctx_create: mem_size/past/int_K outside compiled limits");
        return UPH_ERR_LIMIT;
    }
    HIPCHK(hipSetDevice(uphMapDevice(m)));
    uph_ctx* c = new uph_ctx();
    c->map = m;
    c->device = uphMapDevice(m);
    OptParams& P = c->P;
    P.rho_T = p->rho_T; P.rho_ter = p->rho_ter; P.max_vel = p->max_vel; P.max_acc_lon = p->max_acc_lon; P.max_acc_lat = p->max_acc_lat;
    P.max_kap = p->max_kap; P.min_cxi = p->min_cxi; P.max_sig = p->max_sig; P.use_scaling = p->use_scaling;
    P.beta = p->beta; P.gamma = p->gamma; P.epsilon_con = p->epsilon_con; P.max_iter = p->max_iter;
    P.g_epsilon = p->g_epsilon; P.min_step = p->min_step; P.delta = p->delta;
    P.inner_max_iter = (int)p->inner_max_iter; P.mem_size = p->mem_size; P.past = p->past; P.int_K = p->int_K;
    P.max_linesearch = 64; P.max_step = 1.0e20; P.f_dec_coeff = 1.0e-4; P.s_curv_coeff = 0.9; P.cautious_factor = 1.0e-6; P.machine_prec = 1.0e-16;
    P.no_trial_abandon = 0; P.pad_ = 0;
    finishParams(P);
    c->rho = p->rho;
    {
        std::vector<double> tab;
        buildThomasTable(tab);
        if (c->d_thomas.ensure(tab.size() * sizeof(double))) { delete c; return UPH_ERR_HIP; }
        if (hipMemcpy(c->d_thomas.p, tab.data(), tab.size() * sizeof(double), hipMemcpyHostToDevice) != hipSuccess) { setError("hipMemcpy(thomas table) failed"); c->d_thomas.release(); delete c; return UPH_ERR_HIP; }
    }
    HIPCHK(hipStreamCreateWithFlags(&c->stream, hipStreamNonBlocking));
    {
        int prio_lo = 0, prio_hi = 0;
        hipDeviceGetStreamPriorityRange(&prio_lo, &prio_hi);
        HIPCHK(hipStreamCreateWithPriority(&c->stream2, hipStreamNonBlocking, prio_hi));
    }
    HIPCHK(hipEventCreate(&c->ev2));
    HIPCHK(hipEventCreate(&c->evp0)); HIPCHK(hipEventCreate(&c->evp1));
    HIPCHK(hipEventCreate(&c->ev0));
    HIPCHK(hipEventCreate(&c->ev1));
    *out = c;
    return UPH_OK;
}

void uph_ctx_destroy(uph_ctx* c) {
    if (!c) return;
    hipSetDevice(c->device);
    for (void* p : c->op_allocs) hipFree(p);
    DevBuf* bufs[] = {&c->d_ops, &c->d_desc, &c->d_state, &c->d_x, &c->d_gout, &c->d_dual, &c->d_res, &c->d_scl, &c->d_cxy, &c->d_cyaw,
                      &c->d_hist, &c->d_report, &c->d_order, &c->d_trace, &c->d_x0, &c->d_thomas, &c->d_rsd, &c->d_rs, &c->d_gridmem, &c->d_parammem,
                      &c->d_pen_gxy, &c->d_pen_gyaw, &c->d_pen_out, &c->d_roll_tt, &c->d_roll_traj, &c->d_roll_stage,
                      &c->d_plan_head, &c->d_plan_xy, &c->d_plan_yaw, &c->d_plan_goal, &c->d_plan_rec, &c->d_sw_q, &c->d_sw_out, &c->d_refine_rec, &c->d_win_q,
                      &c->d_win_out, &c->d_delay, &c->d_adopt_rec};
    for (DevBuf* b : bufs) b->release();
    HostBuf* hbufs[] = {&c->h_x, &c->h_cxy, &c->h_cyaw, &c->h_dual, &c->h_res, &c->h_scl};
    for (HostBuf* b : hbufs) b->release();
    if (c->ev0) hipEventDestroy(c->ev0);
    if (c->ev1) hipEventDestroy(c->ev1);
    if (c->stream) hipStreamDestroy(c->stream);
    if (c->stream2) hipStreamDestroy(c->stream2);
    if (c->ev2) hipEventDestroy(c->ev2);
    if (c->evp0) hipEventDestroy(c->evp0);
    if (c->evp1) hipEventDestroy(c->evp1);
    delete c;
}

int uph_ctx_set_lanes(uph_ctx* c, int32_t lanes) {
    if (!c || (lanes != 0 && lanes != 64 && lanes != 128 && lanes != 256 && lanes != 512)) return UPH_ERR_INVALID;
    NOT_ON_FLEET(c, "uph_ctx_set_lanes");
    c->lanes_forced = lanes;
    return UPH_OK;
}
int uph_ctx_set_xcd_locality(uph_ctx* c, int32_t group) { if (!c || group < 0) return UPH_ERR_INVALID; NOT_ON_FLEET(c, "uph_ctx_set_xcd_locality"); c->xcd_group = group; return UPH_OK; }
int uph_ctx_set_wps(uph_ctx* c, int32_t wps) { if (!c || wps < 0 || wps > 2) return UPH_ERR_INVALID; NOT_ON_FLEET(c, "uph_ctx_set_wps"); c->wps_forced = wps; return UPH_OK; }
int uph_ctx_set_sample_precision(uph_ctx* c, int32_t bits) {
    if (!c || (bits != 32 && bits != 64)) { setError("uph_ctx_set_sample_precision: 32 or 64"); return UPH_ERR_INVALID; }
    NOT_ON_FLEET(c, "uph_ctx_set_sample_precision");
    c->sample_f32 = bits == 32;
    return UPH_OK;
}
int uph_ctx_set_rho(uph_ctx* c, double rho) { if (!c) return UPH_ERR_INVALID; NOT_ON_FLEET(c, "uph_ctx_set_rho"); c->rho = rho; return UPH_OK; }
int uph_ctx_set_trial_abandon(uph_ctx* c, int32_t on) { if (!c || (on != 0 && on != 1)) return UPH_ERR_INVALID; NOT_ON_FLEET(c, "uph_ctx_set_trial_abandon"); c->P.no_trial_abandon = on ? 0 : 1; return UPH_OK; }
int uph_ctx_get_rho(uph_ctx* c, double* rho) { if (!c || !rho) return UPH_ERR_INVALID; *rho = c->rho; return UPH_OK; }

int uph_ctx_set_trace(uph_ctx* c, int32_t cap) { if (!c || cap < 0) return UPH_ERR_INVALID; NOT_ON_FLEET(c, "uph_ctx_set_trace"); c->trace_cap = cap; return UPH_OK; }
int uph_ctx_get_trace(uph_ctx* c, double* out ) {
    if (c && c->pending) { setError("an asynchronous solve is in flight on this context: call uph_batch_wait first"); return UPH_ERR_INVALID; }
    if (!c || !out || c->trace_cap_up <= 0 || c->B <= 0) return UPH_ERR_INVALID;
    HIPCHK(hipSetDevice(uphMapDevice(c->map)));
    HIPCHK(hipMemcpy(out, c->d_trace.p, sizeof(double) * (size_t)c->B * c->trace_cap_up, hipMemcpyDeviceToHost));
    return UPH_OK;
}

static void yawTurnKink(const uph_problem& pr, double& turn, double& kink) {
    double prev = pr.init_yaw[0];
    turn = 0.0; kink = 0.0;
    for (int i = 0; i <= pr.n_inner_yaw; i++) {
        const double cur = i < pr.n_inner_yaw ? pr.inner_yaw[i] : pr.end_yaw[0];
        const double dy = std::fabs(cur - prev);
        turn += dy; kink = std::max(kink, dy); prev = cur;
    }
}
static double predictedCostOf(int32_t n_inner_xy, int32_t n_inner_yaw, double turn, double kink) {
    const double n = 2.0 * n_inner_xy + n_inner_yaw + 1.0;
    return std::pow(n, 0.831) * std::exp(0.129 * turn) * std::pow(1.0 + kink, 0.408);
}
static double predictedCost(const uph_problem& pr) {
    double turn, kink;
    yawTurnKink(pr, turn, kink);
    return predictedCostOf(pr.n_inner_xy, pr.n_inner_yaw, turn, kink);
}

static ProblemHead headOf(const uph_problem& q) {
    ProblemHead h;
    h.n_inner_xy = q.n_inner_xy; h.n_inner_yaw = q.n_inner_yaw;
    for (int k = 0; k < 6; k++) { h.init_xy[k] = q.init_xy[k]; h.end_xy[k] = q.end_xy[k]; }
    for (int k = 0; k < 3; k++) { h.init_yaw[k] = q.init_yaw[k]; h.end_yaw[k] = q.end_yaw[k]; }
    h.total_time = q.total_time;
    if (q.n_inner_xy < 0 || q.n_inner_yaw < 0 || (q.n_inner_xy > 0 && !q.inner_xy) || (q.n_inner_yaw > 0 && !q.inner_yaw)) {
        h.refused = UPH_ERR_INVALID; h.why = "uph_batch_upload: negative way-point count or missing way-point array";
        return h;
    }
    for (int d = 0; d < 2; d++) { h.lo[d] = std::min(q.init_xy[d], q.end_xy[d]); h.hi[d] = std::max(q.init_xy[d], q.end_xy[d]); }
    for (int i = 0; i < q.n_inner_xy; i++)
        for (int d = 0; d < 2; d++) { h.lo[d] = std::min(h.lo[d], q.inner_xy[2 * i + d]); h.hi[d] = std::max(h.hi[d], q.inner_xy[2 * i + d]); }
    yawTurnKink(q, h.turn, h.kink);
    return h;
}
static const double ph_inner_xy[2] = {0.3, 0.0}, ph_inner_yaw[1] = {0.0};
static uph_problem placeholderProblem() {
    uph_problem placeholder;
    std::memset(&placeholder, 0, sizeof(placeholder));
    placeholder.n_inner_xy = 1; placeholder.n_inner_yaw = 1; placeholder.inner_xy = ph_inner_xy; placeholder.inner_yaw = ph_inner_yaw;
    placeholder.init_xy[2] = 0.05; placeholder.end_xy[0] = 0.6; placeholder.end_xy[2] = 0.05; placeholder.total_time = 1.44;
    return placeholder;
}

static int admitBatch(uph_ctx* c, int32_t B, const ProblemHead* heads, std::vector<const ProblemHead*>& pp) {
    const int K1 = c->P.int_K + 1, mem = c->P.mem_size;
    c->B = 0;
    c->traj_resident = false;
    c->planned = false;
    c->origin.clear(); c->all_rejected = false;
    int first_rj = 0;
    c->desc.assign(B, TrajDesc());
    int64_t on = 0, os = 0, ocx = 0, ocy = 0, oh = 0;
    size_t lds_d = 0;
    c->lanes = c->lanes_forced ? c->lanes_forced : (B >= 2304 ? 128 : (B <= 256 ? 512 : 256));
    c->wps = c->wps_forced ? c->wps_forced : ((B >= 512) ? 2 : 1);
    c->fp_bytes.assign(B, 0);
    static const ProblemHead placeholder = headOf(placeholderProblem());
    pp.assign(B, nullptr);
    c->rejected.assign(B, 0); c->n_rejected = 0;
    c->end_pose.assign((size_t)3 * B, 0.0);
    c->end_bnd.assign((size_t)9 * B, 0.0);
    const GridDev tg = uphMapGrid(c->map);
    const bool tiled = tg.nx_hold < tg.nx;
    const double tile_lo = tg.origin[0] + tg.x_off * tg.xy_res, tile_hi = tg.origin[0] + (tg.x_off + tg.nx_hold) * tg.xy_res;
    std::string why;
    for (int b = 0; b < B; b++) {
        const ProblemHead& q = heads[b];
        int rj = 0;
        const char* msg = nullptr;
        if (q.refused) { rj = q.refused; msg = q.why; }
        else if (q.n_inner_xy + 1 > UPH_MAX_PIECE_XY || q.n_inner_yaw + 1 > UPH_MAX_PIECE_YAW) { rj = UPH_ERR_LIMIT; msg = "uph_batch_upload: piece count exceeds UPH_MAX_PIECE_*"; }
// ... 342 lines not shown
        s.q = q; s.nxy = nxy[(size_t)q]; s.nyw = nyw[(size_t)q]; s.pad = 0;
        s.row_xy = (int64_t)sq.size();
        const double hx = R / (nxy[(size_t)q] + 1), hy = R / (nyw[(size_t)q] + 1);
        for (int k = 1; k <= s.nxy; k++) sq.push_back(trajQuery(src, b, tc + k * hx));
        s.row_yaw = (int64_t)sq.size();
        for (int k = 1; k <= s.nyw; k++) sq.push_back(trajQuery(src, b, tc + k * hy));
        const double* e = src->end_bnd.data() + (size_t)9 * b;
        s.p_end[0] = e[0]; s.p_end[1] = e[1]; s.yaw_end = e[6]; s.total_time = R;
        rec.push_back(s);
        found.push_back(q);
        ends.insert(ends.end(), e, e + 9);
    }
    r = launchTrajStates(src, sq);
    if (r != UPH_OK) { hipStreamSynchronize(src->stream); return r; }
    std::vector<double> zs((size_t)TRAJ_STATE_COLS * B);
    HIPCHK(hipMemcpyAsync(zs.data(), src->d_sw_out.p, sizeof(double) * TRAJ_STATE_COLS * (size_t)B, hipMemcpyDeviceToHost, src->stream));
    HIPCHK(hipStreamSynchronize(src->stream));
    dst->B = 0;
    dst->traj_resident = false; dst->planned = false; dst->origin.clear(); dst->plan_probs.clear();
    const int F = (int)found.size();
    std::vector<PlanHead> ph((size_t)B);
    if (F > 0) {
        if (dst->d_plan_head.ensure(sizeof(PlanHead) * (size_t)B) || dst->d_plan_xy.ensure(sizeof(double) * 2 * PLAN_SX * (size_t)B) ||
            dst->d_plan_yaw.ensure(sizeof(double) * PLAN_SY * (size_t)B) || dst->d_refine_rec.ensure(sizeof(RefineStage) * (size_t)F))
            return UPH_ERR_HIP;
        HIPCHK(hipMemcpyAsync(dst->d_refine_rec.p, rec.data(), sizeof(RefineStage) * (size_t)F, hipMemcpyHostToDevice, src->stream));
        hipLaunchKernelGGL(uph_refine_stage_kernel, dim3((F + 63) / 64), dim3(64), 0, src->stream, dst->d_refine_rec.as<RefineStage>(), F, src->d_sw_out.as<double>(),
                           dst->d_plan_xy.as<double>(), dst->d_plan_yaw.as<double>(), dst->d_plan_head.as<PlanHead>());
        const hipError_t e = hipGetLastError();
        if (e != hipSuccess) { hipStreamSynchronize(src->stream); setError(std::string("uph_refine_upload: ") + hipGetErrorString(e)); return UPH_ERR_HIP; }
        HIPCHK(hipMemcpyAsync(ph.data(), dst->d_plan_head.p, sizeof(PlanHead) * (size_t)B, hipMemcpyDeviceToHost, src->stream));
        HIPCHK(hipStreamSynchronize(src->stream));
    }
    if (switch_states) std::memcpy(switch_states, zs.data(), sizeof(double) * TRAJ_STATE_COLS * (size_t)B);
    for (int32_t q = 0; q < B; q++) {
        status[q] = rem[(size_t)q] > 0.0 ? UPH_KINO_OK : UPH_REFINE_AT_END; traj_of[q] = -1;
        n_inner_xy[q] = nxy[(size_t)q]; n_inner_yaw[q] = nyw[(size_t)q];
    }
    if (F == 0) { setError("uph_refine_upload: no query left to refine (every switch time at or past its trajectory's end)"); return UPH_ERR_INVALID; }
    std::vector<ProblemHead> heads((size_t)F);
    for (int j = 0; j < F; j++) {
        const int q = found[(size_t)j];
        const PlanHead& g = ph[(size_t)q];
        const double* z = zs.data() + (size_t)TRAJ_STATE_COLS * q;
        const double* e = ends.data() + (size_t)9 * j;
        ProblemHead& h = heads[(size_t)j];
        h.n_inner_xy = nxy[(size_t)q]; h.n_inner_yaw = nyw[(size_t)q];
        for (int k = 0; k < 6; k++) { h.init_xy[k] = z[k]; h.end_xy[k] = e[k]; }
        h.init_yaw[0] = z[9]; h.init_yaw[1] = z[7]; h.init_yaw[2] = z[8];
        for (int k = 0; k < 3; k++) h.end_yaw[k] = e[6 + k];
        h.total_time = rem[(size_t)q];
        for (int d = 0; d < 2; d++) { h.lo[d] = g.lo[d]; h.hi[d] = g.hi[d]; }
        h.turn = g.turn; h.kink = g.kink;
    }
    return uploadStaged(dst, found, heads, traj_of);
}

int uph_plan_staged(uph_ctx* c, int32_t cap_xy, int32_t cap_yaw, double* init_xy, double* end_xy, double* init_yaw, double* end_yaw, double* inner_xy, double* inner_yaw,
                    int32_t* n_inner_xy, int32_t* n_inner_yaw, double* total_time) {
    if (!c || cap_xy < 0 || cap_yaw < 0 || !init_xy || !end_xy || !init_yaw || !end_yaw || !inner_xy || !inner_yaw || !n_inner_xy || !n_inner_yaw || !total_time) {
        setError("uph_plan_staged: bad arguments"); return UPH_ERR_INVALID;
    }
    NOT_ON_FLEET(c, "uph_plan_staged");
    if (c->B <= 0 || !c->planned) { setError("uph_plan_staged: the resident batch did not come from uph_plan_upload"); return UPH_ERR_INVALID; }
    if (c->pending) { setError("uph_plan_staged: an asynchronous solve is in flight (uph_batch_wait first)"); return UPH_ERR_INVALID; }
    HIPCHK(hipSetDevice(uphMapDevice(c->map)));
    int status = UPH_OK;
    for (int j = 0; j < c->B; j++) {
        const ProblemHead& h = c->plan_probs[(size_t)j];
        const int g = c->origin[(size_t)j];
        for (int q = 0; q < 6; q++) { init_xy[(size_t)6 * j + q] = h.init_xy[q]; end_xy[(size_t)6 * j + q] = h.end_xy[q]; }
        for (int q = 0; q < 3; q++) { init_yaw[(size_t)3 * j + q] = h.init_yaw[q]; end_yaw[(size_t)3 * j + q] = h.end_yaw[q]; }
        total_time[j] = h.total_time;
        n_inner_xy[j] = h.n_inner_xy; n_inner_yaw[j] = h.n_inner_yaw;
        const int nx = std::min(std::min(h.n_inner_xy, PLAN_SX), cap_xy), ny = std::min(std::min(h.n_inner_yaw, PLAN_SY), cap_yaw);
        if (h.n_inner_xy > cap_xy || h.n_inner_yaw > cap_yaw || h.n_inner_xy > PLAN_SX || h.n_inner_yaw > PLAN_SY) status = UPH_ERR_LIMIT;
        if (nx > 0) HIPCHK(hipMemcpy(inner_xy + (size_t)2 * cap_xy * j, c->d_plan_xy.as<double>() + (size_t)2 * PLAN_SX * g, sizeof(double) * 2 * nx, hipMemcpyDeviceToHost));
        if (ny > 0) HIPCHK(hipMemcpy(inner_yaw + (size_t)cap_yaw * j, c->d_plan_yaw.as<double>() + (size_t)PLAN_SY * g, sizeof(double) * ny, hipMemcpyDeviceToHost));
    }
    if (status == UPH_ERR_LIMIT) setError("uph_plan_staged: a problem has more way-points than the caller's capacity or the staging's");
    return status;
}

int uph_batch_solve_async(uph_ctx* c) {
    NOT_ON_FLEET(c, "uph_batch_solve_async");
    if (!c || c->B <= 0) { setError("uph_batch_solve_async: no batch uploaded"); return UPH_ERR_INVALID; }
    if (c->pending) { setError("uph_batch_solve_async: the previous asynchronous solve has not been waited for"); return UPH_ERR_INVALID; }
    HIPCHK(hipSetDevice(uphMapDevice(c->map)));
    for (int b = 0; b < c->B; b++) { std::memset(&c->state_host[b], 0, sizeof(TrajState)); c->state_host[b].rho = c->rho; c->state_host[b].scale_fx = 1.0; }
    HIPCHK(hipMemcpyAsync(c->d_state.p, c->state_host.data(), sizeof(TrajState) * c->B, hipMemcpyHostToDevice, c->stream));
    int r = launchSolver(c, 1, 1, true, c->evp0, c->evp1);
    if (r != UPH_OK) { hipStreamSynchronize(c->stream); return r; }
    r = launchSolver(c, 2, 0, true, c->ev0, c->ev1);
    if (r != UPH_OK) { hipStreamSynchronize(c->stream); if (c->stream2) hipStreamSynchronize(c->stream2); return r; }
    c->pending = true;
    return UPH_OK;
}

int uph_batch_wait(uph_ctx* c) {
    NOT_ON_FLEET(c, "uph_batch_wait");
    if (!c || !c->pending) { setError("uph_batch_wait: no asynchronous solve in flight"); return UPH_ERR_INVALID; }
    HIPCHK(hipSetDevice(uphMapDevice(c->map)));
    c->pending = false;
    HIPCHK(hipStreamSynchronize(c->stream));
    float ms = 0.f;
    HIPCHK(hipEventElapsedTime(&ms, c->evp0, c->evp1));
    c->last_prepare_ms = ms;
    HIPCHK(hipEventElapsedTime(&ms, c->ev0, c->ev1));
    c->last_ms = ms;
    int r = refreshStates(c);
    if (r != UPH_OK) return r;
    c->last_evals = c->last_sample_evals = c->last_iters = c->last_hist_bytes = 0;
    for (int q = 0; q < 5; q++) c->last_abandon[q] = 0;
    for (int b = 0; b < c->B; b++) {
        if (c->rejected[b]) continue;
        const TrajState& s = c->state_host[b];
        c->last_evals += s.evals;
        c->last_sample_evals += (int64_t)(s.evals - s.ls_abandoned) * c->desc[b].S;
        c->last_abandon[0] += s.ls_rejected; c->last_abandon[1] += s.ls_guarded; c->last_abandon[2] += s.ls_abandoned;
        c->last_abandon[3] += s.chunks_skipped; c->last_abandon[4] += s.adjoints_skipped;
        c->last_iters += s.lbfgs_iters;
        c->last_hist_bytes += s.hist_reads * 8;
    }
    if (c->B == 1 && !c->rejected[0]) c->rho = c->state_host[0].rho;
    return UPH_OK;
}

int uph_batch_solve(uph_ctx* c) {
    NOT_ON_FLEET(c, "uph_batch_solve");
    const int r = uph_batch_solve_async(c);
    return r != UPH_OK ? r : uph_batch_wait(c);
}

int uph_batch_count(const uph_ctx* c) { return c ? c->B : UPH_ERR_INVALID; }
int uph_batch_origin(const uph_ctx* c, int32_t* idx) {
    NOT_ON_FLEET(c, "uph_batch_origin");
    if (!c || !idx || c->B <= 0) { setError("uph_batch_origin: no batch uploaded"); return UPH_ERR_INVALID; }
    for (int b = 0; b < c->B; b++) idx[b] = c->origin.empty() ? b : c->origin[b];
    return UPH_OK;
}

int uph_batch_stats(uph_ctx* c, double* kernel_ms, int64_t* evals, int64_t* sample_evals, int64_t* lbfgs_iters, int64_t* hist_bytes) {
    if (!c) return UPH_ERR_INVALID;
    NOT_ON_FLEET(c, "uph_batch_stats");
    if (kernel_ms) *kernel_ms = c->last_ms;
    if (evals) *evals = c->last_evals;
    if (sample_evals) *sample_evals = c->last_sample_evals;
    if (lbfgs_iters) *lbfgs_iters = c->last_iters;
    if (hist_bytes) *hist_bytes = c->last_hist_bytes;
    return UPH_OK;
}

int uph_batch_abandon_stats(uph_ctx* c, int64_t* out5) {
    if (!c || !out5) return UPH_ERR_INVALID;
    for (int q = 0; q < 5; q++) out5[q] = c->last_abandon[q];
    return UPH_OK;
}

int uph_batch_prepare_ms(uph_ctx* c, double* ms) { if (!c || !ms) return UPH_ERR_INVALID; *ms = c->last_prepare_ms; return UPH_OK; }

int uph_batch_cycles(uph_ctx* c, long long* out) {
    if (!c || c->B <= 0 || !out) return UPH_ERR_INVALID;
    for (int b = 0; b < c->B; b++) for (int q = 0; q < 16; q++) out[b * 16 + q] = c->state_host[b].cyc[q];
    return UPH_OK;
}

int uph_batch_download(uph_ctx* c, uph_result* results) {
    if (!c || c->B <= 0 || !results) { setError("uph_batch_download: bad arguments"); return UPH_ERR_INVALID; }
    NOT_ON_FLEET(c, "uph_batch_download");
    if (c->pending) { setError("uph_batch_download: an asynchronous solve is in flight (uph_batch_wait first)"); return UPH_ERR_INVALID; }
    HIPCHK(hipSetDevice(uphMapDevice(c->map)));
    int r = refreshStates(c);
    if (r != UPH_OK) return r;
    const GridDev tg = uphMapGrid(c->map);
    const bool tiled = tg.nx_hold < tg.nx;
    const double tile_lo = tg.origin[0] + tg.x_off * tg.xy_res, tile_hi = tg.origin[0] + (tg.x_off + tg.nx_hold) * tg.xy_res;
    bool want_x = tiled, want_cxy = false, want_cyaw = false, want_dual = false, want_res = false, want_scl = false;
    for (int b = 0; b < c->B; b++) {
        const uph_result& o = results[b];
        if (c->rejected[b]) continue;
        want_x |= o.x_final != nullptr; want_cxy |= o.c_xy != nullptr; want_cyaw |= o.c_yaw != nullptr;
        want_dual |= o.lambda != nullptr || o.mu != nullptr; want_res |= o.hx != nullptr || o.gx != nullptr; want_scl |= o.scale_cx != nullptr;
    }
    struct Pull { bool want; HostBuf* h; DevBuf* d; size_t bytes; };
    const Pull pulls[6] = {{want_x, &c->h_x, &c->d_x, (size_t)8 * c->sum_n}, {want_cxy, &c->h_cxy, &c->d_cxy, (size_t)8 * c->sum_cxy},
                           {want_cyaw, &c->h_cyaw, &c->d_cyaw, (size_t)8 * c->sum_cyaw}, {want_dual, &c->h_dual, &c->d_dual, (size_t)8 * 7 * c->sum_S},
                           {want_res, &c->h_res, &c->d_res, (size_t)8 * 7 * c->sum_S}, {want_scl, &c->h_scl, &c->d_scl, (size_t)8 * 7 * c->sum_S}};
    for (const Pull& q : pulls) {
        if (!q.want) continue;
        if (q.h->ensure(q.bytes)) return UPH_ERR_HIP;
        HIPCHK(hipMemcpyAsync(q.h->p, q.d->p, q.bytes, hipMemcpyDeviceToHost, c->stream));
    }
    HIPCHK(hipStreamSynchronize(c->stream));
    const double *x = c->h_x.as<double>(), *cxy = c->h_cxy.as<double>(), *cyaw = c->h_cyaw.as<double>(), *dual = c->h_dual.as<double>(),
                 *res = c->h_res.as<double>(), *scl = c->h_scl.as<double>();
    for (int b = 0; b < c->B; b++) {
        const TrajDesc& t = c->desc[b];
        const TrajState& s = c->state_host[b];
        uph_result& o = results[b];
        if (c->rejected[b]) {
            o.ret_code = UPH_RET_UNSUPPORTED; o.alm_iters = o.lbfgs_iters = o.evals = 0; o.last_lbfgs_ret = c->rejected[b];
            o.cost = o.jerk_cost = o.piece_T_xy = o.piece_T_yaw = 0.0; o.rho_final = c->rho; o.scale_fx = 1.0;
            continue;
        }
        o.ret_code = s.ret_code; o.alm_iters = s.alm_iters; o.lbfgs_iters = s.lbfgs_iters; o.evals = s.evals; o.last_lbfgs_ret = s.last_lbfgs_ret;
        o.cost = s.f; o.jerk_cost = s.jerk_cost; o.piece_T_xy = s.T_xy; o.piece_T_yaw = s.T_yaw; o.rho_final = s.rho; o.scale_fx = s.scale_fx;
        if (tiled) {
            const double* xf = x + t.off_x;
            const double sx = c->frames.empty() ? 0.0 : c->frames[b].shift[0];
            for (int i = 0; i < t.Nxy - 1; i++)
                if ((tg.x_off > 0 && xf[1 + 2 * i] + sx < tile_lo + 2.0 * tg.xy_res) || (tg.x_off + tg.nx_hold < tg.nx && xf[1 + 2 * i] + sx > tile_hi - 2.0 * tg.xy_res)) o.ret_code = UPH_RET_LEFT_TILE;
        }
        if (o.x_final) std::memcpy(o.x_final, x + t.off_x, 8 * t.n);
        if (o.c_xy) std::memcpy(o.c_xy, cxy + t.off_cxy, 8 * 12 * t.Nxy);
        if (!c->frames.empty()) {
            const TrajFrame& f = c->frames[b];
            if (o.x_final) for (int i = 0; i < 2 * (t.Nxy - 1); i++) o.x_final[1 + i] += f.shift[i & 1];
            if (o.c_xy) for (int i = 0; i < t.Nxy; i++) for (int d = 0; d < 2; d++) o.c_xy[12 * i + d] += f.shift[d];
        }
        if (o.c_yaw) std::memcpy(o.c_yaw, cyaw + t.off_cyaw, 8 * 6 * t.Nyaw);
        if (!o.lambda && !o.mu && !o.hx && !o.gx && !o.scale_cx) continue;
        const int S = t.S;
        const double* dl = want_dual ? dual + 7 * t.off_s : nullptr;
        const double* rs = want_res ? res + 7 * t.off_s : nullptr;
        const double* sc = want_scl ? scl + 7 * t.off_s : nullptr;
        for (int i = 0; i < S; i++) {
            if (o.lambda) o.lambda[i] = dl[i];
            if (o.hx) o.hx[i] = rs[i];
            for (int q = 0; q < 6; q++) {
                if (o.mu) o.mu[6 * i + q] = dl[(q + 1) * S + i];
                if (o.gx) o.gx[6 * i + q] = rs[(q + 1) * S + i];
            }
            if (o.scale_cx) for (int q = 0; q < 7; q++) o.scale_cx[7 * i + q] = sc[q * S + i];
        }
    }
    return UPH_OK;
}

// ... 104 lines not shown
            if (lambda) dl[i] = lambda[os + i];
            if (mu) for (int q = 0; q < 6; q++) dl[(q + 1) * S + i] = mu[6 * (os + i) + q];
            if (scale_cx) for (int q = 0; q < 7; q++) sc[q * S + i] = scale_cx[7 * (os + i) + q];
        }
        if (scale_fx) c->state_host[b].scale_fx = scale_fx[b];
        if (rho) c->state_host[b].rho = rho[b];
        os += S;
    }
    HIPCHK(hipMemcpy(c->d_dual.p, dual.data(), 8 * 7 * c->sum_S, hipMemcpyHostToDevice));
    HIPCHK(hipMemcpy(c->d_scl.p, scl.data(), 8 * 7 * c->sum_S, hipMemcpyHostToDevice));
    HIPCHK(hipMemcpy(c->d_state.p, c->state_host.data(), sizeof(TrajState) * c->B, hipMemcpyHostToDevice));
    return UPH_OK;
}

int uph_eval_batch(uph_ctx* c, const double* x_packed, double* f, double* grad_packed, int32_t repeat) {
    NOT_ON_FLEET(c, "uph_eval_batch");
    if (c && c->n_rejected) { setError("packed-array hooks need a batch without unsupported problems (uph_result.ret_code == UPH_RET_UNSUPPORTED)"); return UPH_ERR_INVALID; }
    if (!c || c->B <= 0 || repeat < 1) { setError("uph_eval_batch: bad arguments"); return UPH_ERR_INVALID; }
    HIPCHK(hipSetDevice(uphMapDevice(c->map)));
    if (x_packed) { const int rx = uploadPackedX(c, x_packed); if (rx != UPH_OK) return rx; }
    int r = launchSolver(c, 0, repeat);
    if (r != UPH_OK) return r;
    r = refreshStates(c);
    if (r != UPH_OK) return r;
    if (f) for (int b = 0; b < c->B; b++) f[b] = c->state_host[b].f;
    if (grad_packed) HIPCHK(hipMemcpy(grad_packed, c->d_gout.p, 8 * c->sum_n, hipMemcpyDeviceToHost));
    c->last_evals = (int64_t)c->B * repeat;
    c->last_sample_evals = c->sum_S * repeat;
    c->last_iters = 0; c->last_hist_bytes = 0;
    return UPH_OK;
}

int uph_penalty_batch(uph_ctx* c, int32_t repeat, int32_t store_residuals, double* cost, double* gdcxy_packed, double* gdcyaw_packed, double* gdT2) {
    NOT_ON_FLEET(c, "uph_penalty_batch");
    if (c && c->n_rejected) { setError("packed-array hooks need a batch without unsupported problems (uph_result.ret_code == UPH_RET_UNSUPPORTED)"); return UPH_ERR_INVALID; }
    if (!c || c->B <= 0 || repeat < 1 || repeat > (1 << 20)) { setError("uph_penalty_batch: bad arguments"); return UPH_ERR_INVALID; }
    HIPCHK(hipSetDevice(uphMapDevice(c->map)));
    if (c->d_pen_gxy.ensure(8 * c->sum_cxy) || c->d_pen_gyaw.ensure(8 * c->sum_cyaw) || c->d_pen_out.ensure(8 * 3 * (size_t)c->B)) return UPH_ERR_HIP;
    int r = launchSolver(c, 8, 2 * repeat + (store_residuals ? 1 : 0));
    if (r != UPH_OK) return r;
    if (cost || gdT2) {
        std::vector<double> o3((size_t)3 * c->B);
        HIPCHK(hipMemcpy(o3.data(), c->d_pen_out.p, 8 * o3.size(), hipMemcpyDeviceToHost));
        for (int b = 0; b < c->B; b++) {
            if (cost) cost[b] = o3[3 * (size_t)b];
            if (gdT2) { gdT2[2 * (size_t)b] = o3[3 * (size_t)b + 1]; gdT2[2 * (size_t)b + 1] = o3[3 * (size_t)b + 2]; }
        }
    }
    if (gdcxy_packed) HIPCHK(hipMemcpy(gdcxy_packed, c->d_pen_gxy.p, 8 * c->sum_cxy, hipMemcpyDeviceToHost));
    if (gdcyaw_packed) HIPCHK(hipMemcpy(gdcyaw_packed, c->d_pen_gyaw.p, 8 * c->sum_cyaw, hipMemcpyDeviceToHost));
    c->last_evals = (int64_t)c->B * repeat;
    c->last_sample_evals = c->sum_S * repeat;
    c->last_iters = 0; c->last_hist_bytes = 0;
    return UPH_OK;
}

int uph_microbench_batch(uph_ctx* c, int32_t reps) {
    if (!c || c->B <= 0 || reps < 1) return UPH_ERR_INVALID;
    NOT_ON_FLEET(c, "uph_microbench_batch");
    int r = launchSolver(c, 5, reps);
    if (r != UPH_OK) return r;
    return refreshStates(c);
}

int uph_init_scaling_batch(uph_ctx* c) {
    NOT_ON_FLEET(c, "uph_init_scaling_batch");
    if (!c || c->B <= 0) { setError("uph_init_scaling_batch: no batch uploaded"); return UPH_ERR_INVALID; }
    int r = launchSolver(c, 4, 1);
    if (r != UPH_OK) return r;
    return refreshStates(c);
}

int uph_report_batch(uph_ctx* c, double* out7) {
    NOT_ON_FLEET(c, "uph_report_batch");
    if (!c || c->B <= 0 || !out7) { setError("uph_report_batch: bad arguments"); return UPH_ERR_INVALID; }
    int r = launchSolver(c, 3, 1);
    if (r != UPH_OK) return r;
    HIPCHK(hipMemcpy(out7, c->d_report.p, 8 * 7 * c->B, hipMemcpyDeviceToHost));
    return UPH_OK;
}

static void collectSolveStats(uph_ctx* c) {
    c->last_evals = c->last_sample_evals = c->last_iters = c->last_hist_bytes = 0;
    for (int q = 0; q < 5; q++) c->last_abandon[q] = 0;
    for (int b = 0; b < c->B; b++) {
        if (c->rejected[b]) continue;
        const TrajState& s = c->state_host[b];
        c->last_evals += s.evals;
        c->last_sample_evals += (int64_t)(s.evals - s.ls_abandoned) * c->desc[b].S;
        c->last_abandon[0] += s.ls_rejected; c->last_abandon[1] += s.ls_guarded; c->last_abandon[2] += s.ls_abandoned;
        c->last_abandon[3] += s.chunks_skipped; c->last_abandon[4] += s.adjoints_skipped;
        c->last_iters += s.lbfgs_iters;
        c->last_hist_bytes += s.hist_reads * 8;
    }
}
int uph_batch_set_x(uph_ctx* c, const double* x_packed) {
    NOT_ON_FLEET(c, "uph_batch_set_x");
    if (c && c->pending) { setError("an asynchronous solve is in flight on this context: call uph_batch_wait first"); return UPH_ERR_INVALID; }
    if (c && c->n_rejected) { setError("packed-array hooks need a batch without unsupported problems (uph_result.ret_code == UPH_RET_UNSUPPORTED)"); return UPH_ERR_INVALID; }
    if (!c || c->B <= 0 || !x_packed) { setError("uph_batch_set_x: bad arguments"); return UPH_ERR_INVALID; }
    HIPCHK(hipSetDevice(c->device));
    return uploadPackedX(c, x_packed);
}
int uph_batch_alm_passes(uph_ctx* c, int32_t max_passes) {
    NOT_ON_FLEET(c, "uph_batch_alm_passes");
    if (!c || c->B <= 0 || max_passes < 0) { setError("uph_batch_alm_passes: bad arguments"); return UPH_ERR_INVALID; }
    int r = launchSolver(c, 2, max_passes);
    if (r != UPH_OK) return r;
    r = refreshStates(c);
    if (r != UPH_OK) return r;
    collectSolveStats(c);
    return UPH_OK;
}
int uph_batch_set_lbfgs_state(uph_ctx* c, const double* g, const double* d, const double* pf, const double* lm_s, const double* lm_y, const double* lm_ys, const double* scal5) {
    NOT_ON_FLEET(c, "uph_batch_set_lbfgs_state");
    if (c && c->pending) { setError("an asynchronous solve is in flight on this context: call uph_batch_wait first"); return UPH_ERR_INVALID; }
    if (c && c->n_rejected) { setError("packed-array hooks need a batch without unsupported problems (uph_result.ret_code == UPH_RET_UNSUPPORTED)"); return UPH_ERR_INVALID; }
    if (!c || c->B <= 0 || !g || !d || !pf || !lm_s || !lm_y || !lm_ys || !scal5) { setError("uph_batch_set_lbfgs_state: bad arguments"); return UPH_ERR_INVALID; }
    HIPCHK(hipSetDevice(c->device));
    const int mem = c->P.mem_size;
    if (c->d_rsd.ensure(8 * c->sum_n) || c->d_rs.ensure(8 * 24 * (size_t)c->B)) return UPH_ERR_HIP;
    std::vector<double> hist((size_t)c->sum_hist, 0.0), rs((size_t)24 * c->B, 0.0);
    int64_t off = 0;
    for (int b = 0; b < c->B; b++) {
        const TrajDesc& t = c->desc[b];
        const int rowd = histRowDoubles(t.n), np = 64 * histNQ(t.n);
        for (int j = 0; j < mem; j++) {
            double* row = hist.data() + t.off_hist + (size_t)j * rowd;
            const double ys = lm_ys[(size_t)b * mem + j];
            row[0] = ys; row[1] = 1.0 / ys;
            std::memcpy(row + 2, lm_s + off + (size_t)j * t.n, 8 * t.n);
            std::memcpy(row + 2 + np, lm_y + off + (size_t)j * t.n, 8 * t.n);
        }
        off += (int64_t)mem * t.n;
        for (int q = 0; q < 5; q++) rs[(size_t)24 * b + q] = scal5[5 * b + q];
        for (int q = 0; q < UPH_MAX_PAST; q++) rs[(size_t)24 * b + 8 + q] = pf[(size_t)b * UPH_MAX_PAST + q];
    }
    HIPCHK(hipMemcpy(c->d_hist.p, hist.data(), 8 * c->sum_hist, hipMemcpyHostToDevice));
    HIPCHK(hipMemcpy(c->d_rs.p, rs.data(), 8 * rs.size(), hipMemcpyHostToDevice));
    HIPCHK(hipMemcpy(c->d_gout.p, g, 8 * c->sum_n, hipMemcpyHostToDevice));
    HIPCHK(hipMemcpy(c->d_rsd.p, d, 8 * c->sum_n, hipMemcpyHostToDevice));
    return UPH_OK;
}
int uph_batch_lbfgs_resume(uph_ctx* c, int32_t budget, int32_t finish_pass) {
    NOT_ON_FLEET(c, "uph_batch_lbfgs_resume");
    if (!c || c->B <= 0 || !c->d_rs.p) { setError("uph_batch_lbfgs_resume: no state set"); return UPH_ERR_INVALID; }
    const int bud = budget < 0 ? (1 << 28) : budget;
    int r = launchSolver(c, 7, 2 * bud + (finish_pass ? 1 : 0));
    if (r != UPH_OK) return r;
    r = refreshStates(c);
    if (r != UPH_OK) return r;
    collectSolveStats(c);
    return UPH_OK;
}
int uph_batch_get_lbfgs_state(uph_ctx* c, double* g, double* d, double* pf, double* lm_s, double* lm_y, double* lm_ys, double* scal8) {
    NOT_ON_FLEET(c, "uph_batch_get_lbfgs_state");
    if (c && c->pending) { setError("an asynchronous solve is in flight on this context: call uph_batch_wait first"); return UPH_ERR_INVALID; }
    if (!c || c->B <= 0 || !c->d_rs.p) { setError("uph_batch_get_lbfgs_state: no state set"); return UPH_ERR_INVALID; }
    HIPCHK(hipSetDevice(c->device));
    const int mem = c->P.mem_size;
    std::vector<double> hist((size_t)c->sum_hist), rs((size_t)24 * c->B);
    HIPCHK(hipMemcpy(hist.data(), c->d_hist.p, 8 * c->sum_hist, hipMemcpyDeviceToHost));
    HIPCHK(hipMemcpy(rs.data(), c->d_rs.p, 8 * rs.size(), hipMemcpyDeviceToHost));
    if (g) HIPCHK(hipMemcpy(g, c->d_gout.p, 8 * c->sum_n, hipMemcpyDeviceToHost));
    if (d) HIPCHK(hipMemcpy(d, c->d_rsd.p, 8 * c->sum_n, hipMemcpyDeviceToHost));
    int64_t off = 0;
    for (int b = 0; b < c->B; b++) {
        const TrajDesc& t = c->desc[b];
        const int rowd = histRowDoubles(t.n), np = 64 * histNQ(t.n);
        for (int j = 0; j < mem; j++) {
            const double* row = hist.data() + t.off_hist + (size_t)j * rowd;
            if (lm_ys) lm_ys[(size_t)b * mem + j] = row[0];
            if (lm_s) std::memcpy(lm_s + off + (size_t)j * t.n, row + 2, 8 * t.n);
            if (lm_y) std::memcpy(lm_y + off + (size_t)j * t.n, row + 2 + np, 8 * t.n);
// ... 26 lines not shown
```

### uneven_planner_amd/csrc/uph_common.hpp

```cpp
#pragma once
#include <math.h>
#include <stdint.h>

#if defined(__HIPCC__)
#define UPH_HD __host__ __device__ __forceinline__
#define UPH_NOINLINE __host__ __device__ __attribute__((noinline))
#else
#define UPH_HD inline
#define UPH_NOINLINE __attribute__((noinline))
#endif

#if defined(__HIP_DEVICE_COMPILE__)
#define UPH_AS_GLOBAL(p) ((const __attribute__((address_space(1))) double*)(p))
#else
#define UPH_AS_GLOBAL(p) (p)
#endif

#if defined(UPH_ISA_MARKS) && defined(__HIP_DEVICE_COMPILE__)
#define UPH_MARK(name) asm volatile("; UPHMARK " name)
#else
#define UPH_MARK(name) do { } while (0)
#endif

namespace uph {
// ... 23 lines not shown
    LBFGSERR_INVALID_FDECCOEFF,
    LBFGSERR_INVALID_SCURVCOEFF,
    LBFGSERR_INVALID_MACHINEPREC,
    LBFGSERR_INVALID_MAXLINESEARCH,
    LBFGSERR_INVALID_FUNCVAL,
    LBFGSERR_MINIMUMSTEP,
    LBFGSERR_MAXIMUMSTEP,
    LBFGSERR_MAXIMUMLINESEARCH,
    LBFGSERR_MAXIMUMITERATION,
    LBFGSERR_WIDTHTOOSMALL,
    LBFGSERR_INVALIDPARAMETERS,
    LBFGSERR_INCREASEGRADIENT,
};

struct GridDev {
    int nx, ny, nyaw;
    int x_off, nx_hold;
    int ix_off = 0, iy_off = 0;
    double xy_res, yaw_res, xy_inv, yaw_inv;
    double origin[3], minb[3], maxb[3];
    double lo[3], hi[3];
    double half_xy, half_yaw;
    double gravity;
    const double* cells;
    const float* cells32;
};

struct OptParams {
    double rho_T, rho_ter, max_vel, max_acc_lon, max_acc_lat, max_kap, min_cxi, max_sig;
    int use_scaling;
    double beta, gamma, epsilon_con, max_iter;
    double g_epsilon, min_step, delta;
    int inner_max_iter, mem_size, past, int_K;
    int max_linesearch;
    double max_step, f_dec_coeff, s_curv_coeff, cautious_factor, machine_prec;
    double max_vel2, max_acc_lon2, max_acc_lat2, max_kap2;
    int no_trial_abandon = 0, pad_ = 0;
};

inline void finishGrid(GridDev& g) {
    for (int i = 0; i < 3; i++) { g.lo[i] = g.minb[i] + 1e-4; g.hi[i] = g.maxb[i] - 1e-4; }
    g.half_xy = 0.5 * g.xy_res; g.half_yaw = 0.5 * g.yaw_res;
}
inline void finishParams(OptParams& P) {
    P.max_vel2 = P.max_vel * P.max_vel; P.max_acc_lon2 = P.max_acc_lon * P.max_acc_lon;
    P.max_acc_lat2 = P.max_acc_lat * P.max_acc_lat; P.max_kap2 = P.max_kap * P.max_kap;
}

struct MincoOp {
    int N;
    const double* Wt;
    const double* Wr;
};

constexpr double FRAME_EXTENT = 32.0;
struct TrajFrame {
    double fo[2];
    double lo[2], hi[2];
    double shift[2];
    int ioff[2];
};
inline void applyFrame(GridDev& g, const TrajFrame& f) {
    g.origin[0] = f.fo[0]; g.origin[1] = f.fo[1];
    g.lo[0] = f.lo[0]; g.lo[1] = f.lo[1]; g.hi[0] = f.hi[0]; g.hi[1] = f.hi[1];
    g.ix_off = f.ioff[0]; g.iy_off = f.ioff[1];
}

struct TrajDesc {
    int Nxy, Nyaw, n, S;
    int op_xy, op_yaw;
    int64_t off_x;
    int64_t off_s;
    int64_t off_cxy, off_cyaw;
    int64_t off_hist;
    double init_xy[6], end_xy[6], init_yaw[3], end_yaw[3];
};

struct TrajState {
    double rho, scale_fx;
    double f, jerk_cost, T_xy, T_yaw;
    int ret_code, alm_iters, lbfgs_iters, evals, last_lbfgs_ret, pad;
    long long hist_reads;
    long long cyc[16];
    int ls_rejected, ls_guarded, ls_abandoned, chunks_skipped, adjoints_skipped, pad2;
};

struct BatchDev {
    int B;
    const TrajDesc* desc;
    TrajState* state;
    const MincoOp* ops;
    const double* x0;
    double* x;
    double* gout;
    double* dual;
    double* res;
    double* scl;
    double* cxy;
    double* cyaw;
    double* hist;
    double* rs_d;
    double* rs;
    double* report;
    double* pen_gxy;
    double* pen_gyaw;
    double* pen_out;
    double* trace;
    int trace_cap;
    const int* order;
    const OptParams* params_mem;
    const GridDev* grid_mem;
    int grid_per_traj;
    const double* thomas;
};

#if defined(__HIP_DEVICE_COMPILE__)
UPH_HD void pinv(double& v) { asm volatile("" : "+v"(v)); }
UPH_HD void pinv(float& v) { asm volatile("" : "+v"(v)); }
UPH_HD void pinv(int& v) { asm volatile("" : "+v"(v)); }
#else
UPH_HD void pinv(double&) {}
UPH_HD void pinv(float&) {}
UPH_HD void pinv(int&) {}
#endif
#ifndef UPH_DIET
#define UPH_DIET 0
#endif

UPH_HD double dmax(double a, double b) { return a > b ? a : b; }
UPH_HD double dmin(double a, double b) { return a < b ? a : b; }

UPH_HD double expC2(double tau) { return tau > 0.0 ? ((0.5 * tau + 1.0) * tau + 1.0) : 1.0 / ((0.5 * tau - 1.0) * tau + 1.0); }
UPH_HD double divR(double x, double y, double r) {
    const double q0 = x * r;
    return fma(fma(-q0, y, x), r, q0);
}
UPH_HD void mv2(const double* M, double v0, double v1, double& o0, double& o1) {
    o0 = fma(M[1], v1, M[0] * v0);
    o1 = fma(M[3], v1, M[2] * v0);
}
UPH_HD void submv2(double r0, double r1, const double* M, double p0, double p1, double& o0, double& o1) {
    o0 = fma(-M[1], p1, fma(-M[0], p0, r0));
    o1 = fma(-M[3], p1, fma(-M[2], p0, r1));
}
UPH_HD int histNQ(int n) { return (n + 63) >> 6; }
UPH_HD int histRowDoubles(int n) { return 2 + 128 * histNQ(n); }
constexpr int THOMAS_J = 26;
constexpr int THOMAS_STRIDE = 8;
constexpr int THOMAS_DOUBLES = (THOMAS_J + 1) * THOMAS_STRIDE;
constexpr int THOMAS_KPL = 4;
UPH_HD int knotOff(int q, int ks) { return ks * q + (q >> 2); }
UPH_HD int knotOffJ(int j, int ks) { return ks * j + ((j + 3) >> 2); }
UPH_HD int knotBufDoubles(int nknots, int ks) { return ks * nknots + (nknots >> 2) + 2; }
template <bool ADJ>
UPH_HD void thomasFactors(const double* tab, int j, double* P, double* M1, double* Q, double* M2) {
    const double* e = tab + (j < THOMAS_J ? j : THOMAS_J) * THOMAS_STRIDE;
    const double* en = tab + (j + 1 < THOMAS_J ? j + 1 : THOMAS_J) * THOMAS_STRIDE;
    const double D00 = e[4], D01 = e[5], D10 = e[6], D11 = e[7];
    if (!ADJ) {
        P[0] = 1.0; P[1] = 0.0; P[2] = 0.0; P[3] = 1.0;
        M1[0] = e[0]; M1[1] = e[1]; M1[2] = e[2]; M1[3] = e[3];
        Q[0] = D00; Q[1] = D01; Q[2] = D10; Q[3] = D11;
        M2[0] = fma(8.0, D00, -7.0 * D01); M2[1] = D01 - D00; M2[2] = fma(8.0, D10, -7.0 * D11); M2[3] = D11 - D10;
    } else {
        P[0] = D00; P[1] = D10; P[2] = D01; P[3] = D11;
        const double z = j == 1 ? 0.0 : 1.0;
        M1[0] = z * fma(8.0, D00, -D10); M1[1] = z * fma(-7.0, D00, D10); M1[2] = z * fma(8.0, D01, -D11); M1[3] = z * fma(-7.0, D01, D11);
// ... 111 lines not shown
```

### uneven_planner_amd/csrc/uph_ctx.hpp

```cpp
#pragma once
#include <hip/hip_runtime.h>

#include <map>
#include <string>
#include <vector>

#include "uph_internal.hpp"

using namespace uph;

struct DevBuf {
    void* p = nullptr;
    size_t cap = 0;
    int ensure(size_t bytes) {
        if (bytes <= cap) return 0;
        if (p) hipFree(p);
        p = nullptr; cap = 0;
        size_t want = bytes + bytes / 4 + 256;
        if (hipMalloc(&p, want) != hipSuccess) { setError("hipMalloc failed"); return -1; }
        cap = want;
        return 0;
    }
    void release() { if (p) hipFree(p); p = nullptr; cap = 0; }
    template <class T> T* as() { return (T*)p; }
// ... 10 lines not shown
        if (hipHostMalloc(&p, want, hipHostMallocDefault) != hipSuccess) { setError("hipHostMalloc failed"); return -1; }
        cap = want;
        return 0;
    }
    void release() { if (p) hipHostFree(p); p = nullptr; cap = 0; }
    template <class T> T* as() { return (T*)p; }
};

struct ProblemHead {
    int32_t n_inner_xy = 0, n_inner_yaw = 0;
    int refused = 0;
    const char* why = nullptr;
    double init_xy[6], end_xy[6], init_yaw[3], end_yaw[3], total_time = 0.0;
    double lo[2], hi[2];
    double turn = 0.0, kink = 0.0;
};
struct uph_ctx {
    uph_map* map = nullptr;
    int device = 0;
    OptParams P;
    double rho = 1.0;
    hipStream_t stream = nullptr;
    hipEvent_t ev0 = nullptr, ev1 = nullptr;
    std::map<int, int> op_index;
    std::vector<MincoOp> ops_host;
    std::vector<void*> op_allocs;
    DevBuf d_ops;
    bool ops_dirty = false;
    int B = 0;
    std::vector<TrajDesc> desc;
    std::vector<int> order;
    int64_t sum_n = 0, sum_S = 0, sum_cxy = 0, sum_cyaw = 0, sum_hist = 0;
    size_t lds_bytes = 0;
    size_t lds_big = 0;
    int n_main = 0;
    std::vector<int> rejected;
    int n_rejected = 0;
    bool all_rejected = false;
    std::vector<TrajFrame> frames;
    std::vector<GridDev> grid_host_framed;
    GridDev frames_grid;
    GridDev framed_from;
    bool framed_valid = false;
    std::vector<int> origin;
    bool sample_f32 = false;
    int xcd_group = 0;
    hipStream_t stream2 = nullptr;
    hipEvent_t evp0 = nullptr, evp1 = nullptr;
    bool pending = false;
    hipEvent_t ev2 = nullptr;
    std::vector<size_t> fp_bytes;
    int lanes = 64;
    int lanes_forced = 0;
    int wps = 1;
    int wps_forced = 0;
    DevBuf d_thomas, d_rsd, d_rs, d_gridmem, d_parammem;
    GridDev grid_host;
    DevBuf d_desc, d_state, d_x, d_x0, d_gout, d_dual, d_res, d_scl, d_cxy, d_cyaw, d_hist, d_report, d_order, d_trace;
    DevBuf d_pen_gxy, d_pen_gyaw, d_pen_out;
    DevBuf d_roll_tt, d_roll_traj, d_roll_stage;
    bool traj_resident = false;
    DevBuf d_plan_head, d_plan_xy, d_plan_yaw, d_plan_goal, d_plan_rec;
    bool planned = false;
    std::vector<ProblemHead> plan_probs;
    std::vector<double> end_pose;
    std::vector<double> end_bnd;
    DevBuf d_sw_q, d_sw_out;
    DevBuf d_refine_rec;
    DevBuf d_win_q, d_win_out;
    double last_check_ms = 0.0;
    double last_locate_ms = 0.0;
    double last_sep_ms = 0.0;
    DevBuf d_delay;
    double last_delay_ms = 0.0;
    double last_foot_ms = 0.0;
    double last_foot_check_ms = 0.0;
    double last_clear_check_ms = 0.0;
    int trace_cap = 0;
    int trace_cap_up = 0;
    std::vector<TrajState> state_host;
    HostBuf h_x, h_cxy, h_cyaw, h_dual, h_res, h_scl;
    double last_ms = 0.0, last_prepare_ms = 0.0;
    int64_t last_evals = 0, last_sample_evals = 0, last_iters = 0, last_hist_bytes = 0;
    int64_t last_abandon[5] = {0, 0, 0, 0, 0};
    bool is_fleet = false;
    int fleet_cap_xy = 0, fleet_cap_yaw = 0;
    std::vector<double> fleet_t0;
    DevBuf d_adopt_rec;
    double last_adopt_ms = 0.0;
};
inline bool refusedOnFleet(const uph_ctx* c, const char* who) {
    if (!c || !c->is_fleet) return false;
    setError(std::string(who) + ": the context is a fleet (its slots are filled by uph_fleet_adopt; it takes no upload, solve, evaluation, report, download or batch state)");
    return true;
}
#define NOT_ON_FLEET(c, who)                                  \
    do {                                                      \
        if (refusedOnFleet((c), (who))) return UPH_ERR_INVALID; \
    } while (0)

#define HIPCHK(call)                                                                               \
    do {                                                                                           \
        hipError_t _e = (call);                                                                    \
        if (_e != hipSuccess) {                                                                    \
            setError(std::string(#call) + ": " + hipGetErrorString(_e));                           \
            return UPH_ERR_HIP;                                                                    \
        }                                                                                          \
    } while (0)

int refreshStates(uph_ctx* c);
int syncGridMem(uph_ctx* c, uph::GridDev& grid);

struct SwitchQuery {
    int32_t b, framed;
    double t;
    double shift[2];
};
constexpr int SWITCH_COLS = 9, TRAJ_STATE_COLS = 10;
int checkTrajQueries(const uph_ctx* c, int32_t n, const int32_t* traj, const double* t, const char* who);
SwitchQuery trajQuery(const uph_ctx* c, int32_t b, double t);
int launchTrajStates(uph_ctx* c, const std::vector<SwitchQuery>& sq, int cols = TRAJ_STATE_COLS);
```

Before: 55580.

## Abandon line-search trials early after the first sample chunk using a lower bound

During line-search trial evaluations, the first sample chunk's penalty contribution is summed and published. Together with the jerk cost, a time-penalty lower bound and a dual-term bound computed over chunk 0's multipliers, this gives a lower bound on the trial objective. If that bound already exceeds the Armijo threshold, the remaining chunks and the adjoint are skipped. This adds a cross-wave reduction on chunk 0 and an extra dual-norm reduction per dual update, and relies on the bound being valid so accepted steps are unchanged.

```diff
diff --git a/include/uneven_hip.h b/include/uneven_hip.h
--- a/include/uneven_hip.h
+++ b/include/uneven_hip.h
@@ -221,6 +221,7 @@
 int uph_ctx_set_rho(uph_ctx* c, double rho);
 int uph_ctx_get_rho(uph_ctx* c, double* rho);
 int uph_ctx_set_trial_abandon(uph_ctx* c, int32_t on);
+int uph_ctx_set_chunk0_abandon(uph_ctx* c, int32_t on);
 
 int uph_ctx_set_trace(uph_ctx* c, int32_t cap);
 int uph_ctx_get_trace(uph_ctx* c, double* out);
@@ -237,6 +238,7 @@
 int uph_batch_download(uph_ctx* c, uph_result* results);
 int uph_batch_stats(uph_ctx* c, double* kernel_ms, int64_t* evals, int64_t* sample_evals, int64_t* lbfgs_iters, int64_t* hist_bytes);
 int uph_batch_abandon_stats(uph_ctx* c, int64_t* out5);
+int uph_batch_chunk0_abandoned(uph_ctx* c, int64_t* out);
 
 int uph_batch_prepare_ms(uph_ctx* c, double* ms);
 
diff --git a/uneven_planner_amd/_lib.py b/uneven_planner_amd/_lib.py
--- a/uneven_planner_amd/_lib.py
+++ b/uneven_planner_amd/_lib.py
@@ -124,6 +124,7 @@
     "uph_ctx_set_rho": (C.c_int, [_VP, C.c_double]),
     "uph_ctx_get_rho": (C.c_int, [_VP, DP]),
     "uph_ctx_set_trial_abandon": (C.c_int, [_VP, _I32]),
+    "uph_ctx_set_chunk0_abandon": (C.c_int, [_VP, _I32]),
     "uph_ctx_set_trace": (C.c_int, [_VP, _I32]),
     "uph_ctx_get_trace": (C.c_int, [_VP, DP]),
     "uph_optimize_batch": (C.c_int, [_VP, _I32, C.POINTER(Problem), C.POINTER(Result)]),
@@ -135,6 +136,7 @@
     "uph_batch_stats": (C.c_int, [_VP, DP, C.POINTER(_I64), C.POINTER(_I64), C.POINTER(_I64), C.POINTER(_I64)]),
     "uph_batch_prepare_ms": (C.c_int, [_VP, DP]),
     "uph_batch_abandon_stats": (C.c_int, [_VP, C.POINTER(_I64)]),
+    "uph_batch_chunk0_abandoned": (C.c_int, [_VP, C.POINTER(_I64)]),
     "uph_batch_cycles": (C.c_int, [_VP, C.POINTER(C.c_longlong)]),
     "uph_build_id": (C.c_char_p, []),
     "uph_eval_batch": (C.c_int, [_VP, DP, DP, DP, _I32]),
diff --git a/uneven_planner_amd/alm_traj_opt.py b/uneven_planner_amd/alm_traj_opt.py
--- a/uneven_planner_amd/alm_traj_opt.py
+++ b/uneven_planner_amd/alm_traj_opt.py
@@ -621,6 +621,9 @@
     def set_trial_abandon(self, on):
         _lib.check(self.L.uph_ctx_set_trial_abandon(self.h, 1 if on else 0), "uph_ctx_set_trial_abandon")
 
+    def set_chunk0_abandon(self, on):
+        _lib.check(self.L.uph_ctx_set_chunk0_abandon(self.h, 1 if on else 0), "uph_ctx_set_chunk0_abandon")
+
     def get_rho(self):
         r = C.c_double(0)
         _lib.check(self.L.uph_ctx_get_rho(self.h, C.byref(r)), "uph_ctx_get_rho")
@@ -654,8 +657,10 @@
         _lib.check(self.L.uph_batch_prepare_ms(self.h, C.byref(pm)), "uph_batch_prepare_ms")
         ab = (C.c_int64 * 5)()
         _lib.check(self.L.uph_batch_abandon_stats(self.h, ab), "uph_batch_abandon_stats")
+        c0 = C.c_int64(0)
+        _lib.check(self.L.uph_batch_chunk0_abandoned(self.h, C.byref(c0)), "uph_batch_chunk0_abandoned")
         return dict(kernel_ms=ms.value, prepare_ms=pm.value, evals=v[0].value, sample_evals=v[1].value, lbfgs_iters=v[2].value, hist_bytes=v[3].value,
-                    ls_rejected=ab[0], ls_guarded=ab[1], ls_abandoned=ab[2], chunks_skipped=ab[3], adjoints_skipped=ab[4])
+                    ls_rejected=ab[0], ls_guarded=ab[1], ls_abandoned=ab[2], ls_abandoned_c0=c0.value, chunks_skipped=ab[3], adjoints_skipped=ab[4])
 
     def cycles(self):
         out = np.zeros((max(0, self.L.uph_batch_count(self.h)), 16), dtype=np.int64)
@@ -1383,7 +1388,7 @@
     return method
 
 
-FLEET_REFUSED = ("set_lanes", "set_xcd_locality", "set_wps", "set_sample_precision", "set_rho", "set_trial_abandon", "upload", "solve", "solve_async", "wait", "stats",
+FLEET_REFUSED = ("set_lanes", "set_xcd_locality", "set_wps", "set_sample_precision", "set_rho", "set_trial_abandon", "set_chunk0_abandon", "upload", "solve", "solve_async", "wait", "stats",
                  "cycles", "origin", "download", "optimize_batch", "prepare_boundary", "optimize_boundary", "plan_goals_upload", "plan_goals", "replan_goals_upload",
                  "replan_goals", "refine_upload", "refine", "plan_staged", "optimizeSE2Traj", "getTrajJerkCost", "getMaxVxAxAyCurAttSig", "x0_packed", "eval_batch",
                  "penalty_batch", "init_scaling_batch", "set_state", "set_x", "alm_passes", "set_lbfgs_state", "lbfgs_resume", "get_lbfgs_state", "set_trace", "get_trace")
diff --git a/uneven_planner_amd/csrc/solver_program.hpp b/uneven_planner_amd/csrc/solver_program.hpp
--- a/uneven_planner_amd/csrc/solver_program.hpp
+++ b/uneven_planner_amd/csrc/solver_program.hpp
@@ -13,6 +13,9 @@
 #endif
 #ifndef UPH_STATE_PROBE
 #define UPH_STATE_PROBE(st) do { } while (0)
+#endif
+#ifndef UPH_CHUNK0_PROBE
+#define UPH_CHUNK0_PROBE(R1, thr, mag) do { } while (0)
 #endif
 #ifndef UPH_SCALING_WB
 #define UPH_SCALING_WB 8
@@ -46,6 +49,20 @@
 UPH_HD void sampleChunk(WG& wg, int n, bool first, C compute, P commit) {
     (void)first;
     wg.template accChunk<M>(n, [&](int t, double* acc) { H h; compute(t, acc, h); commit(t, h); });
+}
+#ifndef UPH_CHUNK0_ABANDON
+#define UPH_CHUNK0_ABANDON 1
+#endif
+constexpr int SAMPLE_PUB_LANES = 512;
+template <int M, class H, class WG, class C, class P>
+UPH_HD double sampleChunkPub(WG& wg, int n, bool first, bool pub, C compute, P commit) {
+    (void)first;
+    double cp[SAMPLE_PUB_LANES];
+    wg.template accChunk<M>(n, [&](int t, double* acc) { H h; compute(t, acc, h); commit(t, h); if (pub) cp[t] = acc[0]; });
+    if (!pub) return 0.0;
+    double r[1];
+    wg.template sum<1>(n, r, [&](int t, double* a) { a[0] += cp[t]; });
+    return r[0];
 }
 template <class WG, class F>
 UPH_HD void pforOpen(WG& wg, int n, F f) { wg.pfor(n, f); }
@@ -63,9 +80,9 @@
     double *x, *xp, *g, *gp, *d, *cxy, *cyaw, *Gxy, *Gyaw, *gamxy, *gamyaw, *bt, *rec, *wtab, *ttab, *pf, *hd;
     double* ab;
     int* abn;
-    static constexpr int AB_DOUBLES = 4;
+    static constexpr int AB_DOUBLES = 5;
     double* up;
-    static constexpr int UP_DOUBLES = 6;
+    static constexpr int UP_DOUBLES = 5;
     UPH_HD void tally(int k, bool yes) {
 #if defined(__HIP_DEVICE_COMPILE__)
         if (yes && wg.wave == 0) abn[k] = abn[k] + 1;
@@ -97,19 +114,23 @@
         return (size_t)5 * n + (nvec < td_ ? td_ : nvec) + 2 * (12 * Nxy + 6 * Nyaw) + recd + (size_t)6 * (K + 1) + THOMAS_DOUBLES + MAX_PAST + 8 + 18 + AB_DOUBLES + UP_DOUBLES;
     }
 
+    static UPH_HD int chunkSamples(int CH, int K, int Nxy, int S) {
+#if !defined(UPH_ALIGNED_CHUNKS) || UPH_ALIGNED_CHUNKS
+        const int ppc = CH / (K + 1);
+        if (ppc >= 1 && (Nxy + ppc - 1) / ppc == (S + CH - 1) / CH) return ppc * (K + 1);
+#else
+        (void)K; (void)Nxy; (void)S;
+#endif
+        return CH;
+    }
+
     UPH_HD Solver(WG& w, const GridDev& gr, const OptParams& p, const BatchDev& b, int bi, double* lds)
         : wg(w), grid(gr), P(p), bd(b), td(b.desc[bi]) {
         bidx = bi;
         Nxy = td.Nxy; Nyaw = td.Nyaw; n = td.n; S = td.S; K = P.int_K; mem = P.mem_size;
         inv_k1 = 1.0f / (float)(K + 1);
         CH = wg.size(); CHP = CH + 1; recd = REC_FIELDS * CHP + (CH + 1) / 2;
-        CHS = CH;
-#if !defined(UPH_ALIGNED_CHUNKS) || UPH_ALIGNED_CHUNKS
-        {
-            const int ppc = CH / (K + 1);
-            if (ppc >= 1 && (Nxy + ppc - 1) / ppc == (S + CH - 1) / CH) CHS = ppc * (K + 1);
-        }
-#endif
+        CHS = chunkSamples(CH, K, Nxy, S);
         double* q = lds;
         x = q; q += n; g = q; q += n; d = q; q += n;
         xp = q; q += n; gp = q; q += n;
@@ -141,7 +162,7 @@
         for (int q = 0; q < 16; q++) cyc[q] = 0;
         t_last_eval_end = 0;
         wg.pfor(18 + THOMAS_DOUBLES, [&](int t) {
-            if (t == 0) { ab[0] = 0.0; abn[0] = abn[1] = abn[2] = abn[3] = 0; }
+            if (t == 0) { ab[0] = 0.0; abn[0] = abn[1] = abn[2] = abn[3] = 0; abn[4] = abn[5] = 0; ab[4] = 0.0; }
             if (t < 18) hd[t] = t < 6 ? td.init_xy[t] : (t < 12 ? td.end_xy[t - 6] : (t < 15 ? td.init_yaw[t - 12] : td.end_yaw[t - 15]));
             else ttab[t - 18] = bd.thomas[t - 18];
         });
@@ -857,12 +878,40 @@
         double sm[3] = {0.0, 0.0, 0.0};
         wg.template accBegin<3>();
 #if UPH_CHUNK_OVERLAP
+#if UPH_CHUNK0_ABANDON
+#endif
         for (int s0 = 0; s0 < S; s0 += CHS) {
             const int cnt = S - s0 < CHS ? S - s0 : CHS;
             t0 = wg.clock();
+#if UPH_CHUNK0_ABANDON
+            if (UPH_PHASE_MASK & 2) {
+                const bool pub = STEP && s0 == 0 && S > CHS;
+                const double C0 = sampleChunkPub<3, SampleRec<SR>>(wg, cnt, s0 == 0, pub, [&](int t, double* acc, SampleRec<SR>& h) { sampleCompute<0, SR>(s0 + t, acc, h); },
+                                                                   [&](int t, const SampleRec<SR>& h) { sampleCommit<SR>(t, h); });
+                if (pub && thr < __builtin_huge_val() && ec_omega >= 0.0 && wg.bcast((double)abn[5]) != 0.0) {
+#if UPH_ASIDE_PREP
+                    double eq = wg.bcast(up[3]);
+#else
+                    double eq = expC2(tau);
+#endif
+                    pinv(eq);
+                    const double tau_lb = P.rho_T * eq * scale_fx;
+                    const double lbd = wg.bcast(ab[0]), lbd0 = wg.bcast(ab[4]);
+                    const double R1 = wg.bcast(jerk_cost + tau_lb + C0 - (lbd - lbd0));
+                    const double mag = wg.bcast(fabs(jerk_cost) + fabs(tau_lb) + fabs(C0) + lbd + lbd0);
+                    UPH_CHUNK0_PROBE(R1, thr, mag);
+                    if (R1 > thr + ABANDON_REL * mag && R1 < __builtin_huge_val()) {
+                        tally(4, true);
+                        t_last_eval_end = wg.clock();
+                        return R1;
+                    }
+                }
+            }
+#else
             if (UPH_PHASE_MASK & 2)
                 sampleChunk<3, SampleRec<SR>>(wg, cnt, s0 == 0, [&](int t, double* acc, SampleRec<SR>& h) { sampleCompute<0, SR>(s0 + t, acc, h); },
                                               [&](int t, const SampleRec<SR>& h) { sampleCommit<SR>(t, h); });
+#endif
             t1 = wg.clock(); cyc[1] += t1 - t0;
             if (UPH_PHASE_MASK & 4) scatterChunk<false>(s0, cnt);
             cyc[2] += wg.clock() - t1;
@@ -1144,17 +1193,19 @@
         }
     }
 
-    UPH_HD bool abandonAllowed() const {
-        if (sizeof(SR) != sizeof(double)) return false;
+    UPH_HD int abandonStages() const {
+        if (sizeof(SR) != sizeof(double)) return 0;
 #if defined(__HIP_DEVICE_COMPILE__) && UPH_GRID_FROM_MEM
         typedef const __attribute__((address_space(4))) int* pi_t;
         pi_t pt = (pi_t)(const void*)&bd.params_mem->no_trial_abandon;
         asm volatile("" : "+s"(pt));
-        return *pt == 0;
+        const int sw = *pt;
 #else
-        return P.no_trial_abandon == 0;
-#endif
-    }
+        const int sw = P.no_trial_abandon;
+#endif
+        return (sw & 1) ? 0 : ((sw & 2) ? 1 : 3);
+    }
+    UPH_HD bool abandonAllowed() const { return abandonStages() != 0; }
     static UPH_HD bool noExitAfterRejection(int count, double stp, double mu, double stpmin, double stpmax, int max_linesearch, double machine_prec) {
         return count + 1 < max_linesearch && (stp - mu) >= machine_prec * stp && 0.5 * (mu + stp) >= stpmin && stp <= stpmax;
     }
@@ -1167,7 +1218,18 @@
         const double finit = wg.bcast(f);
         const double dgtest = wg.bcast(P.f_dec_coeff * dginit);
         const double dstest = wg.bcast(P.s_curv_coeff * dginit);
-        const bool on = abandonAllowed();
+        const int stages = abandonStages();
+        const bool on = stages != 0;
+#if UPH_CHUNK0_ABANDON
+        {
+            const int on0 = (stages & 2) != 0 ? 1 : 0;
+#if defined(__HIP_DEVICE_COMPILE__)
+            if (wg.wave == 0) abn[5] = on0;
+#else
+            abn[5] = on0;
+#endif
+        }
+#endif
         const double pst = wg.bcast(P.past > 0 ? P.delta / P.past * (fabs(finit) + 1.0) : 0.0);
         while (true) {
             const double arm = stp * dgtest;
@@ -1299,9 +1361,24 @@
         return ret;
     }
 
-    UPH_HD void setDualBound(double sq) {
+    UPH_HD void setDualBound(double sq, double sq0) {
         const double v = rho > 0.0 ? sq * (0.5 / rho) : __builtin_huge_val();
-        wg.one([&]() { ab[0] = v; });
+        const double v0 = rho > 0.0 ? sq0 * (0.5 / rho) : __builtin_huge_val();
+        wg.one([&]() { ab[0] = v; ab[4] = v0; });
+    }
+    UPH_HD double chunk0Squares() {
+#if UPH_CHUNK0_ABANDON
+        if (S > CHS) {
+            double sq[1];
+            wg.template sum<1>(CHS, sq, [&](int s, double* acc) {
+                double a = 0.0;
+                for (int q = 0; q < 7; q++) { const double v = dual[q * S + s]; a += v * v; }
+                acc[0] += a;
+            });
+            return sq[0];
+        }
+#endif
+        return 0.0;
     }
     UPH_HD void formDualBound() {
         double sq[1];
@@ -1310,7 +1387,7 @@
             for (int q = 0; q < 7; q++) { const double v = dual[q * S + s]; a += v * v; }
             acc[0] += a;
         });
-        setDualBound(sq[0]);
+        setDualBound(sq[0], chunk0Squares());
     }
     UPH_HD void updateDualVars() {
         UPH_MARK("updateDualVars");
@@ -1324,7 +1401,7 @@
             acc[0] += a;
         });
         rho = wg.bcast(dmin((1 + P.gamma) * rho, P.beta));
-        setDualBound(sq[0]);
+        setDualBound(sq[0], chunk0Squares());
     }
     UPH_HD bool judgeConvergence() {
         const double r = rho;
@@ -1340,8 +1417,9 @@
         wg.pfor(1, [&](int) {
             st.T_xy = Txy; st.T_yaw = Tyaw; st.jerk_cost = last_jerk; st.scale_fx = scale_fx; st.rho = rho;
             st.evals = evals; st.hist_reads = hist_reads;
-            st.ls_rejected = abn[0]; st.ls_guarded = abn[1]; st.ls_abandoned = abn[2]; st.adjoints_skipped = abn[3] + abn[2];
-            st.chunks_skipped = abn[2] * ((S + CHS - 1) / CHS);
+            st.ls_rejected = abn[0]; st.ls_guarded = abn[1]; st.ls_abandoned = abn[2]; st.adjoints_skipped = abn[3] + abn[2] + abn[4];
+            st.ls_abandoned_c0 = abn[4];
+            st.chunks_skipped = abn[2] * ((S + CHS - 1) / CHS) + abn[4] * ((S + CHS - 1) / CHS - 1);
 #ifdef UPH_TL_PROF
             for (int q = 0; q < 6; q++) cyc[8 + q] = wg.tl[q];
 #endif
diff --git a/uneven_planner_amd/csrc/unevenhip.hip b/uneven_planner_amd/csrc/unevenhip.hip
--- a/uneven_planner_amd/csrc/unevenhip.hip
+++ b/uneven_planner_amd/csrc/unevenhip.hip
@@ -176,6 +176,29 @@
         if (i < n) commit(i, h);
         bar(0);
     }
+    template <int M, class H, class C, class P>
+    __device__ __forceinline__ double accChunkSplitPub(int n, bool first, bool pub, C compute, P commit) {
+        const int i = ftid();
+        {
+            H h;
+            if (i < n) compute(i, pacc, h);
+            if (!first) bar(3);
+            if (i < n) commit(i, h);
+        }
+        double* r = red + par * (NW * MAXM);
+        if (pub) {
+            const double w = waveSum(pacc[0]);
+            r[wave * MAXM] = w;
+        }
+        bar(0);
+        double t = 0.0;
+        if (pub) {
+            t = r[0];
+#pragma unroll
+            for (int w = 1; w < NW; w++) t += r[w * MAXM];
+        }
+        return uni(t);
+    }
     template <int M>
     __device__ __forceinline__ void accEnd(double* out) {
         double acc[M];
@@ -519,6 +542,8 @@
 
 template <int M, class H, int NT, class C, class P>
 __device__ __forceinline__ void sampleChunk(DevWG<NT>& wg, int n, bool first, C compute, P commit) { wg.template accChunkSplit<M, H>(n, first, compute, commit); }
+template <int M, class H, int NT, class C, class P>
+__device__ __forceinline__ double sampleChunkPub(DevWG<NT>& wg, int n, bool first, bool pub, C compute, P commit) { return wg.template accChunkSplitPub<M, H>(n, first, pub, compute, commit); }
 template <int NT, class F>
 __device__ __forceinline__ void pforOpen(DevWG<NT>& wg, int n, F f) { wg.pforOpen(n, f); }
 
@@ -968,7 +993,8 @@
     return UPH_OK;
 }
 int uph_ctx_set_rho(uph_ctx* c, double rho) { if (!c) return UPH_ERR_INVALID; NOT_ON_FLEET(c, "uph_ctx_set_rho"); c->rho = rho; return UPH_OK; }
-int uph_ctx_set_trial_abandon(uph_ctx* c, int32_t on) { if (!c || (on != 0 && on != 1)) return UPH_ERR_INVALID; NOT_ON_FLEET(c, "uph_ctx_set_trial_abandon"); c->P.no_trial_abandon = on ? 0 : 1; return UPH_OK; }
+int uph_ctx_set_trial_abandon(uph_ctx* c, int32_t on) { if (!c || (on != 0 && on != 1)) return UPH_ERR_INVALID; NOT_ON_FLEET(c, "uph_ctx_set_trial_abandon"); c->P.no_trial_abandon = (c->P.no_trial_abandon & 2) | (on ? 0 : 1); return UPH_OK; }
+int uph_ctx_set_chunk0_abandon(uph_ctx* c, int32_t on) { if (!c || (on != 0 && on != 1)) return UPH_ERR_INVALID; NOT_ON_FLEET(c, "uph_ctx_set_chunk0_abandon"); c->P.no_trial_abandon = (c->P.no_trial_abandon & 1) | (on ? 0 : 2); return UPH_OK; }
 int uph_ctx_get_rho(uph_ctx* c, double* rho) { if (!c || !rho) return UPH_ERR_INVALID; *rho = c->rho; return UPH_OK; }
 
 int uph_ctx_set_trace(uph_ctx* c, int32_t cap) { if (!c || cap < 0) return UPH_ERR_INVALID; NOT_ON_FLEET(c, "uph_ctx_set_trace"); c->trace_cap = cap; return UPH_OK; }
@@ -1477,6 +1503,11 @@
     return status;
 }
 
+static int64_t samplesRun(const uph_ctx* c, int b, const TrajState& s) {
+    const int S = c->desc[b].S, chs = Solver<DevWG<64>>::chunkSamples(c->lanes, c->P.int_K, c->desc[b].Nxy, S);
+    return (int64_t)(s.evals - s.ls_abandoned) * S - (int64_t)s.ls_abandoned_c0 * (S - (chs < S ? chs : S));
+}
+
 int uph_batch_solve_async(uph_ctx* c) {
     NOT_ON_FLEET(c, "uph_batch_solve_async");
     if (!c || c->B <= 0) { setError("uph_batch_solve_async: no batch uploaded"); return UPH_ERR_INVALID; }
@@ -1506,14 +1537,14 @@
     int r = refreshStates(c);
     if (r != UPH_OK) return r;
     c->last_evals = c->last_sample_evals = c->last_iters = c->last_hist_bytes = 0;
-    for (int q = 0; q < 5; q++) c->last_abandon[q] = 0;
+    for (int q = 0; q < 6; q++) c->last_abandon[q] = 0;
     for (int b = 0; b < c->B; b++) {
         if (c->rejected[b]) continue;
         const TrajState& s = c->state_host[b];
         c->last_evals += s.evals;
-        c->last_sample_evals += (int64_t)(s.evals - s.ls_abandoned) * c->desc[b].S;
+        c->last_sample_evals += samplesRun(c, b, s);
         c->last_abandon[0] += s.ls_rejected; c->last_abandon[1] += s.ls_guarded; c->last_abandon[2] += s.ls_abandoned;
-        c->last_abandon[3] += s.chunks_skipped; c->last_abandon[4] += s.adjoints_skipped;
+        c->last_abandon[3] += s.chunks_skipped; c->last_abandon[4] += s.adjoints_skipped; c->last_abandon[5] += s.ls_abandoned_c0;
         c->last_iters += s.lbfgs_iters;
         c->last_hist_bytes += s.hist_reads * 8;
     }
@@ -1549,6 +1580,11 @@
 int uph_batch_abandon_stats(uph_ctx* c, int64_t* out5) {
     if (!c || !out5) return UPH_ERR_INVALID;
     for (int q = 0; q < 5; q++) out5[q] = c->last_abandon[q];
+    return UPH_OK;
+}
+int uph_batch_chunk0_abandoned(uph_ctx* c, int64_t* out) {
+    if (!c || !out) return UPH_ERR_INVALID;
+    *out = c->last_abandon[5];
     return UPH_OK;
 }
 
@@ -1819,14 +1855,14 @@
 
 static void collectSolveStats(uph_ctx* c) {
     c->last_evals = c->last_sample_evals = c->last_iters = c->last_hist_bytes = 0;
-    for (int q = 0; q < 5; q++) c->last_abandon[q] = 0;
+    for (int q = 0; q < 6; q++) c->last_abandon[q] = 0;
     for (int b = 0; b < c->B; b++) {
         if (c->rejected[b]) continue;
         const TrajState& s = c->state_host[b];
         c->last_evals += s.evals;
-        c->last_sample_evals += (int64_t)(s.evals - s.ls_abandoned) * c->desc[b].S;
+        c->last_sample_evals += samplesRun(c, b, s);
         c->last_abandon[0] += s.ls_rejected; c->last_abandon[1] += s.ls_guarded; c->last_abandon[2] += s.ls_abandoned;
-        c->last_abandon[3] += s.chunks_skipped; c->last_abandon[4] += s.adjoints_skipped;
+        c->last_abandon[3] += s.chunks_skipped; c->last_abandon[4] += s.adjoints_skipped; c->last_abandon[5] += s.ls_abandoned_c0;
         c->last_iters += s.lbfgs_iters;
         c->last_hist_bytes += s.hist_reads * 8;
     }
diff --git a/uneven_planner_amd/csrc/uph_common.hpp b/uneven_planner_amd/csrc/uph_common.hpp
--- a/uneven_planner_amd/csrc/uph_common.hpp
+++ b/uneven_planner_amd/csrc/uph_common.hpp
@@ -129,7 +129,7 @@
     int ret_code, alm_iters, lbfgs_iters, evals, last_lbfgs_ret, pad;
     long long hist_reads;
     long long cyc[16];
-    int ls_rejected, ls_guarded, ls_abandoned, chunks_skipped, adjoints_skipped, pad2;
+    int ls_rejected, ls_guarded, ls_abandoned, chunks_skipped, adjoints_skipped, ls_abandoned_c0;
 };
 
 struct BatchDev {
diff --git a/uneven_planner_amd/csrc/uph_ctx.hpp b/uneven_planner_amd/csrc/uph_ctx.hpp
--- a/uneven_planner_amd/csrc/uph_ctx.hpp
+++ b/uneven_planner_amd/csrc/uph_ctx.hpp
@@ -116,7 +116,7 @@
     HostBuf h_x, h_cxy, h_cyaw, h_dual, h_res, h_scl;
     double last_ms = 0.0, last_prepare_ms = 0.0;
     int64_t last_evals = 0, last_sample_evals = 0, last_iters = 0, last_hist_bytes = 0;
-    int64_t last_abandon[5] = {0, 0, 0, 0, 0};
+    int64_t last_abandon[6] = {0, 0, 0, 0, 0, 0};
     bool is_fleet = false;
     int fleet_cap_xy = 0, fleet_cap_yaw = 0;
     std::vector<double> fleet_t0;
```

After: 55250. About the same (-0.6%).
